# nagadomi/nunif

Measured on AMD Instinct MI355X. Metric: input MPix/s, waifu2x swin_unet 2x tiled render (tile 256) of 1080p frames, higher is better.
Workload: dtype f16; 1 GPU; waifu2x swin_unet 2x (art scale2x geometry), tile_size=256, 1080p frame, random-init weights; tile_size=256, tile_batch=45, tiles_per_frame=45, concurrent_streams=2, parallelism=frame-sharded x1

## Files before the change

### include/nunif_hip.h

```cpp
#ifndef NUNIF_HIP_H
#define NUNIF_HIP_H

#include <stddef.h>
#include <stdint.h>

#ifdef __cplusplus
extern "C" {
#endif

#define NUNIF_HIP_ABI_VERSION 1

typedef enum {
    NUNIF_HIP_OK = 0,
    NUNIF_HIP_EINVAL = -1,
    NUNIF_HIP_ENOMEM = -2,
    NUNIF_HIP_EHIP = -3,
    NUNIF_HIP_EMISSING = -4,
    NUNIF_HIP_EUNSUPPORTED = -5
} nunif_hip_status;

int nunif_hip_abi_version(void);
const char *nunif_hip_last_error(void);

typedef struct {
    int32_t x_h, x_w, scale, offset, tile_size, blend_size;
    int32_t y_h, y_w, h_blocks, w_blocks;
    int32_t pad_l, pad_r, pad_t, pad_b, y_buffer_h, y_buffer_w;
    int32_t input_tile_step, output_tile_step;
    int32_t out_tile_size;
} nunif_tile_grid;

int nunif_hip_tile_grid_init(int32_t x_h, int32_t x_w, int32_t scale, int32_t offset, int32_t tile_size,
                             int32_t blend_size, nunif_tile_grid *grid);

int nunif_hip_blend_ramp(int32_t blend_size, float *ramp );

int nunif_hip_gather_tiles(const float *x, float *tiles, const nunif_tile_grid *grid, int32_t channels,
                           int32_t tile_begin, int32_t n_tiles, void *stream);

int nunif_hip_stitch_tiles(const float *tile_out, float *y, const nunif_tile_grid *grid, int32_t channels,
                           void *stream);

typedef struct {
    const char *name;
    const float *data;
    int32_t ndim;
    int64_t shape[4];
} nunif_tensor_desc;

typedef struct nunif_swin_unet nunif_swin_unet;

int nunif_hip_swin_unet_create(const nunif_tensor_desc *tensors, int32_t n_tensors, int32_t scale_factor,
                               nunif_swin_unet **handle);
void nunif_hip_swin_unet_destroy(nunif_swin_unet *handle);

int nunif_hip_swin_unet_forward(nunif_swin_unet *handle, const float *x, float *z, int32_t batch,
                                int32_t tile_size, void *stream);

int nunif_hip_swin_unet_render(nunif_swin_unet *handle, const float *x, float *y, int32_t x_h, int32_t x_w,
                               int32_t tile_size, int32_t batch_size, void *stream);

int nunif_hip_swin_unet_render_tile_rows(nunif_swin_unet *handle, const float *x, int32_t x_h, int32_t x_w,
                                         int32_t tile_size, int32_t batch_size, int32_t row_begin, int32_t row_end,
                                         void *stream);
int nunif_hip_swin_unet_tile_row_band(nunif_swin_unet *handle, int32_t x_h, int32_t x_w, int32_t tile_size,
                                      int32_t tile_row, int32_t row0, int32_t n_rows, float *band, int32_t import_band,
                                      void *stream);
int nunif_hip_swin_unet_stitch_rows(nunif_swin_unet *handle, float *y_band, int32_t x_h, int32_t x_w, int32_t tile_size,
                                    int32_t y_row_begin, int32_t y_row_end, void *stream);

typedef struct {
    int32_t n_win[2];
    int32_t wrap[2];
} nunif_swin_block_extent;
int nunif_hip_swin_unet_tile_extents(const nunif_tile_grid *grid, int32_t tile_index, const int32_t *blocks_per_stage,
                                     const int32_t *shifts, int32_t to_image_fused, nunif_swin_block_extent *out);

typedef struct {
    int32_t adj[6];
    uint32_t bounds;
    uint32_t reserved;
} nunif_swin_tail_group;
int nunif_hip_swin_unet_tail_groups(const nunif_swin_block_extent *ext, int32_t n_tiles, int32_t S, int32_t shift,
                                    nunif_swin_tail_group *out, int64_t cap, int64_t *n_groups, int64_t *n_tokens);

int nunif_hip_swin_unet_tail192_test(nunif_swin_unet *handle, int32_t stage, int32_t block, const void *att, void *x,
                                     int64_t n_tokens, const nunif_swin_tail_group *groups, int64_t n_groups, int64_t n_listed,
                                     int32_t rev, void *stream);

typedef struct nunif_swin_unet_v2 nunif_swin_unet_v2;
int nunif_hip_swin_unet_v2_create(const nunif_tensor_desc *tensors, int32_t n_tensors, int32_t scale_factor,
                                  nunif_swin_unet_v2 **handle);
void nunif_hip_swin_unet_v2_destroy(nunif_swin_unet_v2 *handle);
int nunif_hip_swin_unet_v2_forward(nunif_swin_unet_v2 *handle, const float *x, float *z, int32_t batch, int32_t tile_size,
                                   int32_t clamp01, void *stream);

typedef struct nunif_cunet nunif_cunet;
int nunif_hip_cunet_create(const nunif_tensor_desc *tensors, int32_t n_tensors, int32_t no_clip, nunif_cunet **handle);
void nunif_hip_cunet_destroy(nunif_cunet *handle);
int nunif_hip_cunet_forward(nunif_cunet *handle, const float *x, float *z, int32_t batch, int32_t tile_size,
                            void *stream);
int nunif_hip_cunet_render(nunif_cunet *handle, const float *x, float *y, int32_t x_h, int32_t x_w,
                           int32_t tile_size, int32_t batch_size, void *stream);

int nunif_hip_tta_view(const float *x, float *y, int32_t C, int32_t H, int32_t W, int32_t view, void *stream);
int nunif_hip_tta_merge(const float *const *views, float *out, int32_t C, int32_t H, int32_t W, void *stream);
int nunif_hip_alpha_border_padding(const float *rgb, const float *alpha, float *out, float *work, int32_t H, int32_t W,
                                   int32_t offset, void *stream);

typedef struct {
    int32_t B, H, W;
    double divergence;
    double convergence;
    int32_t fill;
    int32_t synthetic_view;
    int32_t width_base;
    const float *convergence_dev;
} nunif_forward_warp_params;

int nunif_hip_forward_warp(const float *c, const float *depth, float *left, float *right, float *lmask,
                           float *rmask, const nunif_forward_warp_params *params, void *stream);

typedef struct nunif_depth_anything nunif_depth_anything;
int nunif_hip_depth_anything_create(const nunif_tensor_desc *tensors, int32_t n_tensors, nunif_depth_anything **handle);
int nunif_hip_depth_anything_create_ex(const nunif_tensor_desc *tensors, int32_t n_tensors, const int32_t *taps, float max_depth,
                                       nunif_depth_anything **handle);
void nunif_hip_depth_anything_destroy(nunif_depth_anything *handle);
int nunif_hip_depth_anything_forward(nunif_depth_anything *handle, const float *x, const float *pos, float *depth,
                                     int32_t B, int32_t h, int32_t w, void *stream);
int nunif_hip_depth_anything_reset_state(nunif_depth_anything *handle);
int nunif_hip_depth_anything_is_temporal(const nunif_depth_anything *handle);

typedef struct nunif_da_features {
    const void *outconv;
    const void *bottleneck;
    const void *blocks[4];
    int32_t bh, bw, rh[4], rw[4], channels;
} nunif_da_features;
int nunif_hip_depth_anything_forward_features(nunif_depth_anything *handle, const float *x, const float *pos, float *depth,
                                              int32_t B, int32_t h, int32_t w, nunif_da_features *features, void *stream);

typedef struct nunif_zoedepth_head nunif_zoedepth_head;
int nunif_hip_zoedepth_head_create(const nunif_tensor_desc *tensors, int32_t n_tensors, float alpha, float min_temp, float max_temp,
                                   nunif_zoedepth_head **handle);
int nunif_hip_zoedepth_head_forward(nunif_zoedepth_head *handle, const nunif_da_features *features, const float *rel, float *out,
                                    int32_t B, int32_t h, int32_t w, void *stream);
int nunif_hip_zoedepth_head_debug_taps(nunif_zoedepth_head *handle, int32_t tap, float *dst, int32_t *dims, void *stream);
void nunif_hip_zoedepth_head_destroy(nunif_zoedepth_head *handle);
int nunif_hip_zoedepth_pad_normalize(const float *x, float *y, int64_t planes, int32_t h, int32_t w, int32_t left, int32_t right,
                                     int32_t top, int32_t bottom, void *stream);

typedef struct nunif_depth_aa nunif_depth_aa;
int nunif_hip_depth_aa_create(const nunif_tensor_desc *tensors, int32_t n_tensors, nunif_depth_aa **handle);
void nunif_hip_depth_aa_destroy(nunif_depth_aa *handle);
int nunif_hip_depth_aa_forward(nunif_depth_aa *handle, const float *x, float *y, int32_t B, int32_t h, int32_t w,
                               int32_t mode, void *stream);

typedef struct nunif_row_flow nunif_row_flow;
int nunif_hip_row_flow_create(const nunif_tensor_desc *tensors, int32_t n_tensors, nunif_row_flow **handle);
void nunif_hip_row_flow_destroy(nunif_row_flow *handle);
int nunif_hip_row_flow_delta(nunif_row_flow *handle, const float *x, float *delta, int32_t B, int32_t h, int32_t w,
                             int32_t flip, void *stream);

typedef struct nunif_row_flow_v2 nunif_row_flow_v2;
int nunif_hip_row_flow_v2_create(const nunif_tensor_desc *tensors, int32_t n_tensors, nunif_row_flow_v2 **handle);
void nunif_hip_row_flow_v2_destroy(nunif_row_flow_v2 *handle);
int nunif_hip_row_flow_v2_delta(nunif_row_flow_v2 *handle, const float *x, float *delta, int32_t B, int32_t h, int32_t w,
                                int32_t flip, void *stream);
int nunif_hip_row_flow_v2_debug_taps(nunif_row_flow_v2 *handle, const float *x, float *delta, float *feature, float *relu1,
                                     float *relu2, float *relu3, float *non_overlap, float *residual, int32_t B, int32_t h,
                                     int32_t w, int32_t flip, void *stream);

int nunif_hip_delta_warp(const float *c, const float *delta, float *out, int32_t B, int32_t C, int32_t H, int32_t W,
                         int32_t dh, int32_t dw, double delta_scale, int32_t flip, void *stream);

typedef struct nunif_light_inpaint nunif_light_inpaint;
int nunif_hip_light_inpaint_create(const nunif_tensor_desc *tensors, int32_t n_tensors, nunif_light_inpaint **handle);
void nunif_hip_light_inpaint_destroy(nunif_light_inpaint *handle);
int nunif_hip_light_inpaint_infer(nunif_light_inpaint *handle, const float *x, const uint8_t *mask, float *out, int32_t B,
                                  int32_t H, int32_t W, int32_t closing, int32_t inner_iter, int32_t outer_iter, void *stream);
int nunif_hip_light_inpaint_infer_ex(nunif_light_inpaint *handle, const float *x, const uint8_t *mask, float *out, int32_t B,
                                     int32_t H, int32_t W, int32_t closing, int32_t inner_iter, int32_t outer_iter,
                                     int32_t mirror_x, void *stream);

int nunif_hip_anaglyph(const float *left, const float *right, float *out, int32_t H, int32_t W, int32_t mode, void *stream);
int nunif_hip_equirectangular(const float *c, float *out, int32_t C, int32_t h, int32_t w, void *stream);

typedef struct nunif_mlbw nunif_mlbw;
int nunif_hip_mlbw_create(const nunif_tensor_desc *tensors, int32_t n_tensors, nunif_mlbw **handle);
void nunif_hip_mlbw_destroy(nunif_mlbw *handle);
int32_t nunif_hip_mlbw_num_layers(const nunif_mlbw *handle);
int nunif_hip_mlbw_delta(nunif_mlbw *handle, const float *x, float *delta, float *weight, int32_t B, int32_t h, int32_t w,
                         int32_t flip, void *stream);
int32_t nunif_hip_mlbw_has_hole_mask(const nunif_mlbw *handle);
int nunif_hip_mlbw_delta_mask(nunif_mlbw *handle, const float *x, float *delta, float *weight, float *mask_logits, int32_t B,
                              int32_t h, int32_t w, int32_t flip, void *stream);
int nunif_hip_hole_mask_postprocess(const float *logits, uint8_t *mask, float *work, int32_t B, int32_t h, int32_t w,
                                    int32_t H, int32_t W, float threshold, int32_t inner_iter, int32_t outer_iter, float *z,
                                    int32_t C, void *stream);

int nunif_hip_delta_weight_warp(const float *c, const float *delta, const float *weight, float *out, int32_t B, int32_t C,
                                int32_t H, int32_t W, int32_t dh, int32_t dw, int32_t L, double delta_scale, int32_t flip,
                                void *stream);

int nunif_hip_backward_warp(const float *c, const float *depth, float *left, float *right, int32_t B, int32_t C,
                            int32_t H, int32_t W, int32_t dh, int32_t dw, double divergence, double convergence,
                            int32_t synthetic_view, void *stream, const float *convergence_dev);

int nunif_hip_resize_aa(const float *x, float *y, float *tmp, int64_t planes, int32_t h_in, int32_t w_in,
                        int32_t h_out, int32_t w_out, int32_t bicubic, int32_t align_corners, int32_t clamp01,
                        const float *mean3, const float *std3, void *stream);

int64_t nunif_hip_dilate_edge_work_floats(int32_t B, int32_t H, int32_t W);
int nunif_hip_dilate_edge(const float *x, float *y, float *work, int32_t B, int32_t H, int32_t W, int32_t n_x,
                          int32_t n_y, void *stream);

int nunif_hip_minmax_normalize(const float *x, float *y, float *minmax, int32_t B, int64_t n_per, void *stream);

int nunif_hip_minmax(const float *x, float *minmax_keys, int32_t B, int64_t n_per, void *stream);
int nunif_hip_ema_scaler_push(float *state, const float *minmax_keys, int32_t ring_size, int64_t count, int32_t filled,
                              int32_t first, double decay, void *stream);
int nunif_hip_ema_scaler_ring_minmax(float *state, int32_t ring_size, void *stream);
int nunif_hip_range_normalize(const float *x, float *y, const float *lohi, int64_t n, int32_t max_mode, void *stream);

int nunif_hip_make_input_planes(const float *depth, float *out, int32_t B, int32_t H, int32_t W, double divergence_value,
                                double convergence_value, int32_t border_pix, void *stream, const float *convergence_dev);

int nunif_hip_stack(const void *const *srcs, int32_t n, int64_t bytes_each, void *dst, void *stream);

int nunif_hip_mask_morphology(const float *in, float *out, float *work, int32_t B, int32_t H, int32_t W, int32_t op,
                              int32_t n_a, int32_t n_b, void *stream);

int nunif_hip_reflection_pad2d(const float *x, float *y, int64_t planes, int32_t H, int32_t W, int32_t left, int32_t right,
                               int32_t top, int32_t bottom, void *stream);
int nunif_hip_depth_postprocess(const float *x, float *y, int64_t n, float max_dist, int32_t to_disparity, float eps,
                                int32_t negate, void *stream);

int nunif_hip_frame_to_tensor(const void *frame, float *chw, int32_t H, int32_t W, int32_t bits, void *stream);
int nunif_hip_stereo_to_frame(const float *left, const float *right, void *frame, int32_t H, int32_t W,
                              int32_t layout, int32_t bits, void *stream);
int nunif_hip_stereo_compose(const float *left, const float *right, float *out, int32_t H, int32_t W,
                             int32_t layout, void *stream);

int nunif_hip_rgb_noise(float *out, int32_t planes, int32_t H, int32_t W, int32_t level, int32_t component, uint64_t seed,
                        uint64_t counter, void *stream);
int nunif_hip_apply_rgb_noise(const float *rgb, const float *noise, float *out, int64_t n, double strength, double gamma,
                              int32_t light_decay, double light_decay_strength, void *stream);
int nunif_hip_grain_blend(float *buf, const float *noise, int64_t n, double speed, int32_t first, void *stream);
int nunif_hip_grain_video_step(const float *rgb, float *noise_buffer, void *frame, int32_t H, int32_t W, int32_t bits,
                               int32_t level, uint64_t seed, uint64_t counter, double speed, int32_t first, double strength,
                               double gamma, int32_t light_decay, double light_decay_strength, void *stream);
int nunif_hip_frame_to_tensor_rot(const void *frame, float *chw, int32_t H, int32_t W, int32_t bits, int32_t turns,
                                  void *stream);

int nunif_hip_map_depth(const float *x, float *y, int64_t n, int32_t kind, double p0, double p1, void *stream);

typedef struct nunif_transnetv2 nunif_transnetv2;
int nunif_hip_transnetv2_create(const nunif_tensor_desc *tensors, int32_t n_tensors, int32_t filters,
                                nunif_transnetv2 **handle);
void nunif_hip_transnetv2_destroy(nunif_transnetv2 *handle);
int nunif_hip_transnetv2_forward(nunif_transnetv2 *handle, const float *frames, int32_t B, int32_t T, float *one_hot,
                                 float *many_hot, float *sigmoid_out, void *stream);

typedef struct nunif_sod_v1 nunif_sod_v1;
int nunif_hip_sod_v1_create(const nunif_tensor_desc *tensors, int32_t n_tensors, int32_t net_size, nunif_sod_v1 **handle);
void nunif_hip_sod_v1_destroy(nunif_sod_v1 *handle);
int64_t nunif_hip_sod_v1_workspace_floats(int32_t B);
int nunif_hip_sod_v1_forward(nunif_sod_v1 *handle, const float *rgb, int32_t H, int32_t W, const float *depth, int32_t h,
                             int32_t w, int32_t B, float *workspace, float *saliency, float *depth_scaled, void *stream);
int nunif_hip_sod_v1_entry(const float *rgb, int32_t H, int32_t W, const float *depth, int32_t h, int32_t w, int32_t B,
                           float *x6, float *depth_scaled, void *stream);
int nunif_hip_sod_v1_debug_taps(nunif_sod_v1 *handle, const float *workspace, int32_t B, const char *name, float *out,
                                int64_t capacity, int64_t *shape4, void *stream);
int nunif_hip_sod_v1_depth_position(const float *saliency, const float *depth, int32_t B, int64_t n, double pos, float *out,
                                    void *stream);
int nunif_hip_sod_v1_ema(const float *z, float *out, int32_t B, float *state, double decay, uint64_t reset_mask, void *stream);

typedef struct nunif_superpoint nunif_superpoint;
int nunif_hip_superpoint_create(const nunif_tensor_desc *tensors, int32_t n_tensors, nunif_superpoint **handle);
void nunif_hip_superpoint_destroy(nunif_superpoint *handle);
int nunif_hip_superpoint_forward(nunif_superpoint *handle, const float *image, int32_t B, int32_t C, int32_t H, int32_t W,
                                 int32_t nms_radius, int32_t remove_borders, float threshold, float *keypoints,
                                 float *kp_scores, int32_t *counts, void *stream);
int nunif_hip_superpoint_debug_taps(nunif_superpoint *handle, const char *name, float *out, int64_t capacity, int64_t *shape4,
                                    void *stream);
int nunif_hip_superpoint_sample(nunif_superpoint *handle, int32_t b, const float *keypoints, int32_t n, float *out,
                                void *stream);

int64_t nunif_hip_superpoint_keypoints_work_floats(int32_t B, int32_t H, int32_t W);
int nunif_hip_superpoint_keypoints(const float *scores, int32_t B, int32_t H, int32_t W, int32_t nms_radius,
                                   int32_t remove_borders, float threshold, float *work, float *nms_out, float *keypoints,
                                   float *kp_scores, int32_t *counts, void *stream);

int nunif_hip_sample_descriptors(const float *keypoints, int32_t n, const float *dense, int32_t h, int32_t w, int32_t C,
                                 int32_t stride, float *out, void *stream);

int nunif_hip_superpoint_match(const float *d1, int32_t n1, const float *d2, int32_t n2, int32_t D, void *work, int64_t *index,
                               float *max_similarity, void *stream);

int nunif_hip_affine_warp(const float *x, const float *params, float *out, int32_t B, int32_t C, int32_t H, int32_t W,
                          int32_t padding_mode, void *stream);

typedef struct nunif_outpaint nunif_outpaint;
int nunif_hip_outpaint_create(const nunif_tensor_desc *tensors, int32_t n_tensors, nunif_outpaint **handle);
void nunif_hip_outpaint_destroy(nunif_outpaint *handle);
int64_t nunif_hip_outpaint_work_bytes(int32_t B, int32_t H, int32_t W, int32_t max_size);
int nunif_hip_outpaint_infer(nunif_outpaint *handle, const float *x, const uint8_t *mask, int32_t B, int32_t H, int32_t W,
                             int32_t max_size, int32_t mode, float *out, void *work, void *stream);
int nunif_hip_outpaint_debug_taps(nunif_outpaint *handle, const void *work, int32_t B, int32_t H, int32_t W, int32_t max_size,
                                  const char *name, float *out, int64_t capacity, int64_t *shape4, void *stream);
int nunif_hip_outpaint_buffer_step(const float *frames, const float *coarse, float *buffer, const uint8_t *reset,
                                   double buffer_decay, int32_t B, int32_t H, int32_t W, float *out, uint8_t *mask0,
                                   void *stream);

int nunif_hip_autocrop_stats(const float *x, int32_t B, int32_t H, int32_t W, int32_t flat, int32_t passes,
                             int32_t *border_count_tb, int32_t *border_count_lr, void *work, int64_t work_bytes, void *stream);
int nunif_hip_autocrop_debug_stats(const float *x, int32_t B, int32_t H, int32_t W, int32_t flat, int32_t passes,
                                   int32_t *border_count_tb, int32_t *border_count_lr, void *work, int64_t work_bytes,
                                   float *row_a, float *row_b, float *col_a, float *col_b, void *stream);
int nunif_hip_autocrop_crop_pad(const float *src, float *dst, int64_t N, int32_t sH, int32_t sW, int32_t dH, int32_t dW,
                                int32_t y0, int32_t x0, int32_t pad_top, int32_t pad_left, int32_t win_h, int32_t win_w,
                                float pad_value, void *stream);

int nunif_hip_jpeg_quant_tables(int32_t quality, uint8_t *luma, uint8_t *chroma);
int64_t nunif_hip_jpeg_header(int32_t H, int32_t W, int32_t quality, int32_t subsampling, int32_t restart_mcus, uint8_t *out,
                              int64_t capacity);
int64_t nunif_hip_jpeg_max_bytes(int32_t H, int32_t W, int32_t subsampling, int32_t restart_mcus);
int64_t nunif_hip_jpeg_workspace_bytes(int32_t B, int32_t H, int32_t W, int32_t subsampling, int32_t restart_mcus);
int nunif_hip_jpeg_encode(const float *rgb, int32_t B, int32_t H, int32_t W, int32_t quality, int32_t subsampling,
                          int32_t restart_mcus, uint8_t *out, int64_t capacity, int32_t *out_len, void *workspace, void *stream);
int nunif_hip_jpeg_debug_coefficients(const float *rgb, int32_t B, int32_t H, int32_t W, int32_t quality, int32_t subsampling,
                                      int16_t *coef, void *stream);

typedef struct nunif_hdr2sdr_params {
    double exposure, white_point, saturation_gain;
} nunif_hdr2sdr_params;
int nunif_hip_hdr2sdr(const void *src, void *dst, int32_t H, int32_t W, int32_t trc, int32_t colorspace,
                      const nunif_hdr2sdr_params *params, int32_t form, void *stream);
int nunif_hip_hdr2sdr_constants(int32_t trc, int32_t colorspace, const nunif_hdr2sdr_params *params, float *matrix,
                                float *hable_white);

typedef struct nunif_pixfmt_planes {
    void *data[3];
    int64_t pitch[3];
} nunif_pixfmt_planes;
int nunif_hip_yuv_to_tensor(const nunif_pixfmt_planes *src, int32_t format, int32_t H, int32_t W, int32_t matrix,
                            int32_t full_range, int32_t form, float *dst, void *frame, void *stream);
int nunif_hip_tensor_to_yuv(const float *src, int32_t H, int32_t W, int32_t format, int32_t matrix, int32_t full_range,
                            const nunif_pixfmt_planes *dst, void *stream);
int nunif_hip_pixfmt_constants(int32_t matrix, int32_t full_range, int32_t bits, int32_t direction, float *coefficients,
                               float *offsets);

int nunif_hip_yuv_hdr_to_tensor(const nunif_pixfmt_planes *src, int32_t format, int32_t H, int32_t W, int32_t full_range,
                                int32_t trc, int32_t colorspace, const nunif_hdr2sdr_params *params, int32_t form,
                                void *dst, void *stream);

typedef struct nunif_cliqa nunif_cliqa;
int nunif_hip_cliqa_create(const nunif_tensor_desc *tensors, int32_t n_tensors, int32_t kind, nunif_cliqa **handle);
void nunif_hip_cliqa_destroy(nunif_cliqa *handle);
int64_t nunif_hip_cliqa_workspace_bytes(nunif_cliqa *handle, int32_t B, int32_t H, int32_t W, int32_t group);
int nunif_hip_cliqa_forward(nunif_cliqa *handle, const float *x, int32_t B, int32_t H, int32_t W, int32_t group, void *workspace,
                            int64_t workspace_bytes, float *out0, float *out1, void *stream);
int nunif_hip_cliqa_debug_taps(nunif_cliqa *handle, const float *x, int32_t B, int32_t H, int32_t W, int32_t group,
                               void *workspace, int64_t workspace_bytes, float *out0, float *out1, void *tap1, void *tap2,
                               void *tap3, float *head_maps, void *stream);
int nunif_hip_cliqa_select_patches(const float *image, int32_t H, int32_t W, int32_t patch_size, int32_t num_patches,
                                   float *scores, int64_t *indices, float *patches, void *stream);

int64_t nunif_hip_png_header(int32_t H, int32_t W, int32_t form, const char *const *text_keys, const char *const *text_values,
                             int32_t n_text, uint8_t *out, int64_t capacity);
int64_t nunif_hip_png_max_bytes(int32_t H, int32_t W, int32_t form, int32_t stripe_rows);
int64_t nunif_hip_png_workspace_bytes(int32_t B, int32_t H, int32_t W, int32_t form, int32_t stripe_rows);
int nunif_hip_png_encode(const void *src, int32_t form, int32_t B, int32_t H, int32_t W, int32_t stripe_rows, uint8_t *out,
                         int64_t capacity, int32_t *out_len, void *workspace, void *stream);
int nunif_hip_png_debug_filtered(const void *src, int32_t form, int32_t B, int32_t H, int32_t W, uint8_t *filtered, void *stream);
int nunif_hip_png_debug_codes(const void *src, int32_t form, int32_t B, int32_t H, int32_t W, int32_t stripe_rows, int32_t *hist,
                              int32_t *lengths, void *workspace, void *stream);
int nunif_hip_png_encode_planes(const float *colour, const float *alpha, int32_t colour_channels, int32_t form, int32_t B, int32_t H,
                                int32_t W, int32_t stripe_rows, uint8_t *out, int64_t capacity, int32_t *out_len, void *workspace,
                                void *stream);
int nunif_hip_png_debug_filtered_planes(const float *colour, const float *alpha, int32_t colour_channels, int32_t form, int32_t B,
                                        int32_t H, int32_t W, uint8_t *filtered, void *stream);

int64_t nunif_hip_da3_disparity_workspace_bytes(int32_t B, int32_t H, int32_t W);
int nunif_hip_da3_disparity(const float *depth, const float *sky, int32_t B, int32_t H, int32_t W, double sky_thresh, double shift,
                            int32_t raw_output, float *out, void *workspace, int64_t workspace_bytes, void *stream);
int nunif_hip_da3_disparity_debug_stats(const void *workspace, int32_t B, float *stats, int32_t *counts, void *stream);
int64_t nunif_hip_da3mono_features_workspace_bytes(int32_t B, int32_t H, int32_t W);
int nunif_hip_da3mono_features(const float *depth, int32_t B, int32_t H, int32_t W, const int64_t *ranks, float *out,
                               void *workspace, int64_t workspace_bytes, void *stream);
typedef struct nunif_da3mono nunif_da3mono;
int nunif_hip_da3mono_create(const nunif_tensor_desc *tensors, int32_t n_tensors, nunif_da3mono **handle);
void nunif_hip_da3mono_destroy(nunif_da3mono *handle);
int64_t nunif_hip_da3mono_workspace_bytes(int32_t B, int32_t H, int32_t W);
int nunif_hip_da3mono_forward(nunif_da3mono *handle, const float *depth, int32_t B, int32_t H, int32_t W, const int64_t *ranks,
                              float *out, void *workspace, int64_t workspace_bytes, void *stream);

int nunif_hip_swin_unet_debug_taps(nunif_swin_unet *handle, int32_t enable);
int nunif_hip_swin_unet_get_tap(nunif_swin_unet *handle, int32_t index, char *name, int32_t name_cap,
                                void *host_dst, int64_t cap_bytes, int64_t *nbytes);
int nunif_hip_cunet_debug_taps(nunif_cunet *handle, int32_t enable);
int nunif_hip_cunet_get_tap(nunif_cunet *handle, int32_t index, char *name, int32_t name_cap,
                            void *host_dst, int64_t cap_bytes, int64_t *nbytes);

int nunif_hip_profile_enable(int32_t on);
typedef struct { char name[48]; double total_ms; int64_t launches; double flops; double bytes; } nunif_prof_record;
int nunif_hip_profile_read(nunif_prof_record *out, int32_t cap, int32_t reset);

#ifdef __cplusplus
}
#endif
#endif
```

### nunif_amd/_hip.py

```python
import ctypes
import os

_HERE = os.path.dirname(os.path.abspath(__file__))
LIB_PATH = os.environ.get("NUNIF_HIP_LIB") or os.path.join(_HERE, "libnunif_hip.so")

c_void_p, c_int32, c_int64, c_float, c_char_p, c_double, c_uint64 = (
    ctypes.c_void_p, ctypes.c_int32, ctypes.c_int64, ctypes.c_float, ctypes.c_char_p, ctypes.c_double, ctypes.c_uint64)


class NunifHipError(RuntimeError):
    def __init__(self, status, message):
        super().__init__(f"libnunif_hip error {status}: {message}")
        self.status = status


class TileGrid(ctypes.Structure):
    _fields_ = [(n, c_int32) for n in (
        "x_h", "x_w", "scale", "offset", "tile_size", "blend_size",
        "y_h", "y_w", "h_blocks", "w_blocks",
        "pad_l", "pad_r", "pad_t", "pad_b", "y_buffer_h", "y_buffer_w",
        "input_tile_step", "output_tile_step", "out_tile_size")]

    def as_config(self):
        return {"y_h": self.y_h, "y_w": self.y_w, "h_blocks": self.h_blocks, "w_blocks": self.w_blocks,
                "pad": (self.pad_l, self.pad_r, self.pad_t, self.pad_b),
                "y_buffer_h": self.y_buffer_h, "y_buffer_w": self.y_buffer_w,
                "input_tile_step": self.input_tile_step, "output_tile_step": self.output_tile_step}


class SwinBlockExtent(ctypes.Structure):
    _fields_ = [("n_win", c_int32 * 2), ("wrap", c_int32 * 2)]


class SwinTailGroup(ctypes.Structure):
    _fields_ = [("adj", c_int32 * 6), ("bounds", ctypes.c_uint32), ("reserved", ctypes.c_uint32)]

    def tokens(self):
        cnt = (self.bounds >> 25) & 31
        firsts = [0] + [(self.bounds >> (5 * p)) & 31 for p in range(5)]
        return [self.adj[max(p for p in range(6) if firsts[p] <= r)] + r for r in range(cnt)]


class TensorDesc(ctypes.Structure):
    _fields_ = [("name", c_char_p), ("data", c_void_p), ("ndim", c_int32), ("shape", c_int64 * 4)]


class ForwardWarpParams(ctypes.Structure):
    _fields_ = [("B", c_int32), ("H", c_int32), ("W", c_int32), ("divergence", c_double), ("convergence", c_double),
                ("fill", c_int32), ("synthetic_view", c_int32), ("width_base", c_int32), ("convergence_dev", c_void_p)]


class Hdr2SdrParams(ctypes.Structure):
    _fields_ = [("exposure", c_double), ("white_point", c_double), ("saturation_gain", c_double)]


class PixfmtPlanes(ctypes.Structure):
    _fields_ = [("data", c_void_p * 3), ("pitch", c_int64 * 3)]


class DaFeatures(ctypes.Structure):
    _fields_ = [("outconv", c_void_p), ("bottleneck", c_void_p), ("blocks", c_void_p * 4), ("bh", c_int32), ("bw", c_int32),
                ("rh", c_int32 * 4), ("rw", c_int32 * 4), ("channels", c_int32)]


class ProfRecord(ctypes.Structure):
    _fields_ = [("name", ctypes.c_char * 48), ("total_ms", c_double), ("launches", c_int64),
                ("flops", c_double), ("bytes", c_double)]


SIGNATURES = {
    "nunif_hip_abi_version": (c_int32, []),
    "nunif_hip_last_error": (c_char_p, []),
    "nunif_hip_tile_grid_init": (c_int32, [c_int32] * 6 + [ctypes.POINTER(TileGrid)]),
    "nunif_hip_blend_ramp": (c_int32, [c_int32, ctypes.POINTER(c_float)]),
    "nunif_hip_gather_tiles": (c_int32, [c_void_p, c_void_p, ctypes.POINTER(TileGrid), c_int32, c_int32, c_int32, c_void_p]),
    "nunif_hip_stitch_tiles": (c_int32, [c_void_p, c_void_p, ctypes.POINTER(TileGrid), c_int32, c_void_p]),
    "nunif_hip_swin_unet_create": (c_int32, [ctypes.POINTER(TensorDesc), c_int32, c_int32, ctypes.POINTER(c_void_p)]),
    "nunif_hip_swin_unet_destroy": (None, [c_void_p]),
    "nunif_hip_swin_unet_forward": (c_int32, [c_void_p, c_void_p, c_void_p, c_int32, c_int32, c_void_p]),
    "nunif_hip_swin_unet_render": (c_int32, [c_void_p, c_void_p, c_void_p, c_int32, c_int32, c_int32, c_int32, c_void_p]),
    "nunif_hip_swin_unet_render_tile_rows": (c_int32, [c_void_p, c_void_p, c_int32, c_int32, c_int32, c_int32, c_int32, c_int32, c_void_p]),
    "nunif_hip_swin_unet_tile_row_band": (c_int32, [c_void_p, c_int32, c_int32, c_int32, c_int32, c_int32, c_int32, c_void_p, c_int32, c_void_p]),
    "nunif_hip_swin_unet_stitch_rows": (c_int32, [c_void_p, c_void_p, c_int32, c_int32, c_int32, c_int32, c_int32, c_void_p]),
    "nunif_hip_swin_unet_tile_extents": (c_int32, [ctypes.POINTER(TileGrid), c_int32, ctypes.POINTER(c_int32), ctypes.POINTER(c_int32),
                                                   c_int32, ctypes.POINTER(SwinBlockExtent)]),
    "nunif_hip_swin_unet_tail_groups": (c_int32, [ctypes.POINTER(SwinBlockExtent), c_int32, c_int32, c_int32,
                                                  ctypes.POINTER(SwinTailGroup), c_int64, ctypes.POINTER(c_int64), ctypes.POINTER(c_int64)]),
    "nunif_hip_swin_unet_tail192_test": (c_int32, [c_void_p, c_int32, c_int32, c_void_p, c_void_p, c_int64, c_void_p, c_int64, c_int64,
                                                   c_int32, c_void_p]),
    "nunif_hip_swin_unet_v2_create": (c_int32, [ctypes.POINTER(TensorDesc), c_int32, c_int32, ctypes.POINTER(c_void_p)]),
    "nunif_hip_swin_unet_v2_destroy": (None, [c_void_p]),
    "nunif_hip_swin_unet_v2_forward": (c_int32, [c_void_p, c_void_p, c_void_p, c_int32, c_int32, c_int32, c_void_p]),
    "nunif_hip_cunet_create": (c_int32, [ctypes.POINTER(TensorDesc), c_int32, c_int32, ctypes.POINTER(c_void_p)]),
    "nunif_hip_cunet_destroy": (None, [c_void_p]),
    "nunif_hip_cunet_forward": (c_int32, [c_void_p, c_void_p, c_void_p, c_int32, c_int32, c_void_p]),
    "nunif_hip_cunet_render": (c_int32, [c_void_p, c_void_p, c_void_p, c_int32, c_int32, c_int32, c_int32, c_void_p]),
    "nunif_hip_forward_warp": (c_int32, [c_void_p, c_void_p, c_void_p, c_void_p, c_void_p, c_void_p,
                                         ctypes.POINTER(ForwardWarpParams), c_void_p]),
    "nunif_hip_backward_warp": (c_int32, [c_void_p, c_void_p, c_void_p, c_void_p] + [c_int32] * 6 +
                                [c_double, c_double, c_int32, c_void_p, c_void_p]),
    "nunif_hip_row_flow_create": (c_int32, [ctypes.POINTER(TensorDesc), c_int32, ctypes.POINTER(c_void_p)]),
    "nunif_hip_row_flow_destroy": (None, [c_void_p]),
    "nunif_hip_row_flow_delta": (c_int32, [c_void_p, c_void_p, c_void_p, c_int32, c_int32, c_int32, c_int32, c_void_p]),
    "nunif_hip_row_flow_v2_create": (c_int32, [ctypes.POINTER(TensorDesc), c_int32, ctypes.POINTER(c_void_p)]),
    "nunif_hip_row_flow_v2_destroy": (None, [c_void_p]),
    "nunif_hip_row_flow_v2_delta": (c_int32, [c_void_p, c_void_p, c_void_p, c_int32, c_int32, c_int32, c_int32, c_void_p]),
    "nunif_hip_row_flow_v2_debug_taps": (c_int32, [c_void_p] * 9 + [c_int32] * 4 + [c_void_p]),
    "nunif_hip_delta_warp": (c_int32, [c_void_p, c_void_p, c_void_p] + [c_int32] * 6 + [c_double, c_int32, c_void_p]),
    "nunif_hip_mlbw_create": (c_int32, [ctypes.POINTER(TensorDesc), c_int32, ctypes.POINTER(c_void_p)]),
    "nunif_hip_mlbw_destroy": (None, [c_void_p]),
    "nunif_hip_mlbw_num_layers": (c_int32, [c_void_p]),
    "nunif_hip_mlbw_delta": (c_int32, [c_void_p, c_void_p, c_void_p, c_void_p, c_int32, c_int32, c_int32, c_int32, c_void_p]),
    "nunif_hip_light_inpaint_create": (c_int32, [ctypes.POINTER(TensorDesc), c_int32, ctypes.POINTER(c_void_p)]),
    "nunif_hip_light_inpaint_destroy": (None, [c_void_p]),
    "nunif_hip_light_inpaint_infer": (c_int32, [c_void_p, c_void_p, c_void_p, c_void_p] + [c_int32] * 6 + [c_void_p]),
    "nunif_hip_light_inpaint_infer_ex": (c_int32, [c_void_p, c_void_p, c_void_p, c_void_p] + [c_int32] * 7 + [c_void_p]),
    "nunif_hip_anaglyph": (c_int32, [c_void_p, c_void_p, c_void_p, c_int32, c_int32, c_int32, c_void_p]),
    "nunif_hip_equirectangular": (c_int32, [c_void_p, c_void_p, c_int32, c_int32, c_int32, c_void_p]),
    "nunif_hip_mlbw_has_hole_mask": (c_int32, [c_void_p]),
    "nunif_hip_mlbw_delta_mask": (c_int32, [c_void_p, c_void_p, c_void_p, c_void_p, c_void_p, c_int32, c_int32, c_int32, c_int32,
                                            c_void_p]),
    "nunif_hip_hole_mask_postprocess": (c_int32, [c_void_p, c_void_p, c_void_p] + [c_int32] * 5 + [c_float, c_int32, c_int32,
                                                  c_void_p, c_int32, c_void_p]),
    "nunif_hip_delta_weight_warp": (c_int32, [c_void_p, c_void_p, c_void_p, c_void_p] + [c_int32] * 7 +
                                    [c_double, c_int32, c_void_p]),
    "nunif_hip_depth_aa_create": (c_int32, [ctypes.POINTER(TensorDesc), c_int32, ctypes.POINTER(c_void_p)]),
    "nunif_hip_depth_aa_destroy": (None, [c_void_p]),
    "nunif_hip_depth_aa_forward": (c_int32, [c_void_p, c_void_p, c_void_p, c_int32, c_int32, c_int32, c_int32, c_void_p]),
    "nunif_hip_depth_anything_create": (c_int32, [ctypes.POINTER(TensorDesc), c_int32, ctypes.POINTER(c_void_p)]),
    "nunif_hip_depth_anything_create_ex": (c_int32, [ctypes.POINTER(TensorDesc), c_int32, ctypes.POINTER(c_int32), ctypes.c_float,
                                                     ctypes.POINTER(c_void_p)]),
    "nunif_hip_depth_anything_destroy": (None, [c_void_p]),
    "nunif_hip_depth_anything_forward": (c_int32, [c_void_p, c_void_p, c_void_p, c_void_p, c_int32, c_int32, c_int32, c_void_p]),
    "nunif_hip_depth_anything_reset_state": (c_int32, [c_void_p]),
    "nunif_hip_depth_anything_is_temporal": (c_int32, [c_void_p]),
    "nunif_hip_depth_anything_forward_features": (c_int32, [c_void_p, c_void_p, c_void_p, c_void_p, c_int32, c_int32, c_int32,
                                                            ctypes.POINTER(DaFeatures), c_void_p]),
    "nunif_hip_zoedepth_head_create": (c_int32, [ctypes.POINTER(TensorDesc), c_int32, c_float, c_float, c_float,
                                                 ctypes.POINTER(c_void_p)]),
    "nunif_hip_zoedepth_head_forward": (c_int32, [c_void_p, ctypes.POINTER(DaFeatures), c_void_p, c_void_p, c_int32, c_int32,
                                                  c_int32, c_void_p]),
    "nunif_hip_zoedepth_head_debug_taps": (c_int32, [c_void_p, c_int32, c_void_p, ctypes.POINTER(c_int32), c_void_p]),
    "nunif_hip_zoedepth_head_destroy": (None, [c_void_p]),
    "nunif_hip_zoedepth_pad_normalize": (c_int32, [c_void_p, c_void_p, c_int64] + [c_int32] * 6 + [c_void_p]),
    "nunif_hip_tta_view": (c_int32, [c_void_p, c_void_p, c_int32, c_int32, c_int32, c_int32, c_void_p]),
    "nunif_hip_tta_merge": (c_int32, [ctypes.POINTER(c_void_p), c_void_p, c_int32, c_int32, c_int32, c_void_p]),
    "nunif_hip_alpha_border_padding": (c_int32, [c_void_p, c_void_p, c_void_p, c_void_p, c_int32, c_int32, c_int32, c_void_p]),
    "nunif_hip_resize_aa": (c_int32, [c_void_p, c_void_p, c_void_p, c_int64] + [c_int32] * 7 +
                            [ctypes.POINTER(c_float), ctypes.POINTER(c_float), c_void_p]),
    "nunif_hip_dilate_edge": (c_int32, [c_void_p, c_void_p, c_void_p] + [c_int32] * 5 + [c_void_p]),
    "nunif_hip_dilate_edge_work_floats": (ctypes.c_int64, [c_int32, c_int32, c_int32]),
    "nunif_hip_minmax_normalize": (c_int32, [c_void_p, c_void_p, c_void_p, c_int32, c_int64, c_void_p]),
    "nunif_hip_mask_morphology": (c_int32, [c_void_p, c_void_p, c_void_p] + [c_int32] * 6 + [c_void_p]),
    "nunif_hip_reflection_pad2d": (c_int32, [c_void_p, c_void_p, c_int64, c_int32, c_int32, c_int32, c_int32, c_int32, c_int32,
                                             c_void_p]),
    "nunif_hip_depth_postprocess": (c_int32, [c_void_p, c_void_p, c_int64, c_float, c_int32, c_float, c_int32, c_void_p]),
    "nunif_hip_frame_to_tensor": (c_int32, [c_void_p, c_void_p, c_int32, c_int32, c_int32, c_void_p]),
    "nunif_hip_stereo_to_frame": (c_int32, [c_void_p, c_void_p, c_void_p, c_int32, c_int32, c_int32, c_int32, c_void_p]),
    "nunif_hip_stereo_compose": (c_int32, [c_void_p, c_void_p, c_void_p, c_int32, c_int32, c_int32, c_void_p]),
    "nunif_hip_rgb_noise": (c_int32, [c_void_p, c_int32, c_int32, c_int32, c_int32, c_int32, c_uint64, c_uint64, c_void_p]),
    "nunif_hip_apply_rgb_noise": (c_int32, [c_void_p, c_void_p, c_void_p, c_int64, c_double, c_double, c_int32, c_double, c_void_p]),
    "nunif_hip_grain_blend": (c_int32, [c_void_p, c_void_p, c_int64, c_double, c_int32, c_void_p]),
    "nunif_hip_grain_video_step": (c_int32, [c_void_p, c_void_p, c_void_p, c_int32, c_int32, c_int32, c_int32, c_uint64, c_uint64,
                                             c_double, c_int32, c_double, c_double, c_int32, c_double, c_void_p]),
    "nunif_hip_frame_to_tensor_rot": (c_int32, [c_void_p, c_void_p, c_int32, c_int32, c_int32, c_int32, c_void_p]),
    "nunif_hip_map_depth": (c_int32, [c_void_p, c_void_p, c_int64, c_int32, c_double, c_double, c_void_p]),
    "nunif_hip_transnetv2_create": (c_int32, [ctypes.POINTER(TensorDesc), c_int32, c_int32, ctypes.POINTER(c_void_p)]),
    "nunif_hip_transnetv2_destroy": (None, [c_void_p]),
    "nunif_hip_transnetv2_forward": (c_int32, [c_void_p, c_void_p, c_int32, c_int32, c_void_p, c_void_p, c_void_p, c_void_p]),
    "nunif_hip_sod_v1_create": (c_int32, [ctypes.POINTER(TensorDesc), c_int32, c_int32, ctypes.POINTER(c_void_p)]),
    "nunif_hip_sod_v1_destroy": (None, [c_void_p]),
    "nunif_hip_sod_v1_workspace_floats": (c_int64, [c_int32]),
    "nunif_hip_sod_v1_forward": (c_int32, [c_void_p, c_void_p, c_int32, c_int32, c_void_p, c_int32, c_int32, c_int32, c_void_p,
                                           c_void_p, c_void_p, c_void_p]),
    "nunif_hip_sod_v1_entry": (c_int32, [c_void_p, c_int32, c_int32, c_void_p, c_int32, c_int32, c_int32, c_void_p, c_void_p,
                                         c_void_p]),
    "nunif_hip_sod_v1_debug_taps": (c_int32, [c_void_p, c_void_p, c_int32, c_char_p, c_void_p, c_int64, ctypes.POINTER(c_int64),
                                              c_void_p]),
    "nunif_hip_sod_v1_depth_position": (c_int32, [c_void_p, c_void_p, c_int32, c_int64, c_double, c_void_p, c_void_p]),
    "nunif_hip_sod_v1_ema": (c_int32, [c_void_p, c_void_p, c_int32, c_void_p, c_double, c_uint64, c_void_p]),
    "nunif_hip_superpoint_create": (c_int32, [ctypes.POINTER(TensorDesc), c_int32, ctypes.POINTER(c_void_p)]),
    "nunif_hip_superpoint_destroy": (None, [c_void_p]),
    "nunif_hip_superpoint_forward": (c_int32, [c_void_p, c_void_p] + [c_int32] * 6 + [c_float, c_void_p, c_void_p, c_void_p,
                                              c_void_p]),
    "nunif_hip_superpoint_debug_taps": (c_int32, [c_void_p, c_char_p, c_void_p, c_int64, ctypes.POINTER(c_int64), c_void_p]),
    "nunif_hip_superpoint_sample": (c_int32, [c_void_p, c_int32, c_void_p, c_int32, c_void_p, c_void_p]),
    "nunif_hip_superpoint_keypoints_work_floats": (c_int64, [c_int32, c_int32, c_int32]),
    "nunif_hip_superpoint_keypoints": (c_int32, [c_void_p] + [c_int32] * 5 + [c_float] + [c_void_p] * 6),
    "nunif_hip_sample_descriptors": (c_int32, [c_void_p, c_int32, c_void_p] + [c_int32] * 4 + [c_void_p, c_void_p]),
    "nunif_hip_superpoint_match": (c_int32, [c_void_p, c_int32, c_void_p, c_int32, c_int32, c_void_p, c_void_p, c_void_p,
                                            c_void_p]),
    "nunif_hip_affine_warp": (c_int32, [c_void_p, c_void_p, c_void_p] + [c_int32] * 5 + [c_void_p]),
    "nunif_hip_outpaint_create": (c_int32, [ctypes.POINTER(TensorDesc), c_int32, ctypes.POINTER(c_void_p)]),
    "nunif_hip_outpaint_destroy": (None, [c_void_p]),
    "nunif_hip_outpaint_work_bytes": (c_int64, [c_int32] * 4),
    "nunif_hip_outpaint_infer": (c_int32, [c_void_p, c_void_p, c_void_p] + [c_int32] * 5 + [c_void_p, c_void_p, c_void_p]),
    "nunif_hip_outpaint_debug_taps": (c_int32, [c_void_p, c_void_p] + [c_int32] * 4 + [c_char_p, c_void_p, c_int64,
                                                ctypes.POINTER(c_int64), c_void_p]),
    "nunif_hip_outpaint_buffer_step": (c_int32, [c_void_p] * 4 + [c_double] + [c_int32] * 3 + [c_void_p] * 3),
    "nunif_hip_autocrop_stats": (c_int32, [c_void_p] + [c_int32] * 5 + [c_void_p, c_void_p, c_void_p, c_int64, c_void_p]),
    "nunif_hip_autocrop_debug_stats": (c_int32, [c_void_p] + [c_int32] * 5 + [c_void_p, c_void_p, c_void_p, c_int64] +
                                       [c_void_p] * 5),
    "nunif_hip_autocrop_crop_pad": (c_int32, [c_void_p, c_void_p, c_int64] + [c_int32] * 10 + [c_float, c_void_p]),
    "nunif_hip_jpeg_quant_tables": (c_int32, [c_int32, c_void_p, c_void_p]),
    "nunif_hip_jpeg_header": (c_int64, [c_int32] * 5 + [c_void_p, c_int64]),
    "nunif_hip_jpeg_max_bytes": (c_int64, [c_int32] * 4),
    "nunif_hip_jpeg_workspace_bytes": (c_int64, [c_int32] * 5),
    "nunif_hip_jpeg_encode": (c_int32, [c_void_p] + [c_int32] * 6 + [c_void_p, c_int64, c_void_p, c_void_p, c_void_p]),
    "nunif_hip_jpeg_debug_coefficients": (c_int32, [c_void_p] + [c_int32] * 5 + [c_void_p, c_void_p]),
    "nunif_hip_png_header": (c_int64, [c_int32] * 3 + [c_void_p, c_void_p, c_int32, c_void_p, c_int64]),
    "nunif_hip_png_max_bytes": (c_int64, [c_int32] * 4),
    "nunif_hip_png_workspace_bytes": (c_int64, [c_int32] * 5),
    "nunif_hip_png_encode": (c_int32, [c_void_p] + [c_int32] * 5 + [c_void_p, c_int64, c_void_p, c_void_p, c_void_p]),
    "nunif_hip_png_debug_filtered": (c_int32, [c_void_p] + [c_int32] * 4 + [c_void_p, c_void_p]),
    "nunif_hip_png_debug_codes": (c_int32, [c_void_p] + [c_int32] * 5 + [c_void_p] * 4),
    "nunif_hip_png_encode_planes": (c_int32, [c_void_p, c_void_p] + [c_int32] * 6 + [c_void_p, c_int64, c_void_p, c_void_p, c_void_p]),
    "nunif_hip_png_debug_filtered_planes": (c_int32, [c_void_p, c_void_p] + [c_int32] * 5 + [c_void_p, c_void_p]),
    "nunif_hip_hdr2sdr": (c_int32, [c_void_p, c_void_p, c_int32, c_int32, c_int32, c_int32, ctypes.POINTER(Hdr2SdrParams), c_int32,
                                    c_void_p]),
    "nunif_hip_hdr2sdr_constants": (c_int32, [c_int32, c_int32, ctypes.POINTER(Hdr2SdrParams), ctypes.POINTER(c_float),
                                              ctypes.POINTER(c_float)]),
    "nunif_hip_yuv_to_tensor": (c_int32, [ctypes.POINTER(PixfmtPlanes)] + [c_int32] * 6 + [c_void_p, c_void_p, c_void_p]),
    "nunif_hip_tensor_to_yuv": (c_int32, [c_void_p] + [c_int32] * 5 + [ctypes.POINTER(PixfmtPlanes), c_void_p]),
    "nunif_hip_pixfmt_constants": (c_int32, [c_int32] * 4 + [ctypes.POINTER(c_float), ctypes.POINTER(c_float)]),
    "nunif_hip_yuv_hdr_to_tensor": (c_int32, [ctypes.POINTER(PixfmtPlanes)] + [c_int32] * 6 + [ctypes.POINTER(Hdr2SdrParams), c_int32,
                                                                                                c_void_p, c_void_p]),
    "nunif_hip_cliqa_create": (c_int32, [ctypes.POINTER(TensorDesc), c_int32, c_int32, ctypes.POINTER(c_void_p)]),
    "nunif_hip_cliqa_destroy": (None, [c_void_p]),
    "nunif_hip_cliqa_workspace_bytes": (c_int64, [c_void_p] + [c_int32] * 4),
    "nunif_hip_cliqa_forward": (c_int32, [c_void_p, c_void_p] + [c_int32] * 4 + [c_void_p, c_int64] + [c_void_p] * 3),
    "nunif_hip_cliqa_debug_taps": (c_int32, [c_void_p, c_void_p] + [c_int32] * 4 + [c_void_p, c_int64] + [c_void_p] * 7),
    "nunif_hip_cliqa_select_patches": (c_int32, [c_void_p] + [c_int32] * 4 + [c_void_p] * 4),
    "nunif_hip_da3_disparity_workspace_bytes": (c_int64, [c_int32] * 3),
    "nunif_hip_da3_disparity": (c_int32, [c_void_p, c_void_p] + [c_int32] * 3 + [c_double, c_double, c_int32, c_void_p, c_void_p,
                                                                                 c_int64, c_void_p]),
    "nunif_hip_da3_disparity_debug_stats": (c_int32, [c_void_p, c_int32, c_void_p, c_void_p, c_void_p]),
    "nunif_hip_da3mono_features_workspace_bytes": (c_int64, [c_int32] * 3),
    "nunif_hip_da3mono_features": (c_int32, [c_void_p] + [c_int32] * 3 + [c_void_p, c_void_p, c_void_p, c_int64, c_void_p]),
    "nunif_hip_da3mono_create": (c_int32, [ctypes.POINTER(TensorDesc), c_int32, ctypes.POINTER(c_void_p)]),
    "nunif_hip_da3mono_destroy": (None, [c_void_p]),
    "nunif_hip_da3mono_workspace_bytes": (c_int64, [c_int32] * 3),
    "nunif_hip_da3mono_forward": (c_int32, [c_void_p, c_void_p] + [c_int32] * 3 + [c_void_p, c_void_p, c_void_p, c_int64, c_void_p]),
    "nunif_hip_swin_unet_debug_taps":(c_int32, [c_void_p, c_int32]),
    "nunif_hip_swin_unet_get_tap": (c_int32, [c_void_p, c_int32, c_char_p, c_int32, c_void_p, c_int64,
                                              ctypes.POINTER(c_int64)]),
    "nunif_hip_cunet_debug_taps": (c_int32, [c_void_p, c_int32]),
    "nunif_hip_cunet_get_tap": (c_int32, [c_void_p, c_int32, c_char_p, c_int32, c_void_p, c_int64,
                                          ctypes.POINTER(c_int64)]),
    "nunif_hip_minmax": (c_int32, [c_void_p, c_void_p, c_int32, c_int64, c_void_p]),
    "nunif_hip_ema_scaler_push": (c_int32, [c_void_p, c_void_p, c_int32, c_int64, c_int32, c_int32, c_double, c_void_p]),
    "nunif_hip_ema_scaler_ring_minmax": (c_int32, [c_void_p, c_int32, c_void_p]),
    "nunif_hip_range_normalize": (c_int32, [c_void_p, c_void_p, c_void_p, c_int64, c_int32, c_void_p]),
    "nunif_hip_make_input_planes": (c_int32, [c_void_p, c_void_p, c_int32, c_int32, c_int32, c_double, c_double, c_int32, c_void_p, c_void_p]),
    "nunif_hip_stack": (c_int32, [ctypes.POINTER(c_void_p), c_int32, c_int64, c_void_p, c_void_p]),
    "nunif_hip_profile_enable": (c_int32, [c_int32]),
    "nunif_hip_profile_read": (c_int32, [ctypes.POINTER(ProfRecord), c_int32, c_int32]),
}

_lib = None


def lib():
    global _lib
    if _lib is None:
        import torch
        if not os.path.exists(LIB_PATH):
            raise RuntimeError(
                f"{LIB_PATH} not found: the HIP engine is not built. Run `python -m nunif_amd.build` "
                "(there is no CPU fallback).")
        handle = ctypes.CDLL(LIB_PATH)
        for name, (restype, argtypes) in SIGNATURES.items():
            fn = getattr(handle, name)
            fn.restype = restype
            fn.argtypes = argtypes
        _lib = handle
    return _lib


def check(status):
    if status != 0:
        raise NunifHipError(status, lib().nunif_hip_last_error().decode("utf-8", "replace"))


def current_stream_ptr(device=None):
    import torch
    return c_void_p(torch.cuda.current_stream(device).cuda_stream)


def tile_grid(x_h, x_w, scale, offset, tile_size, blend_size):
    g = TileGrid()
    check(lib().nunif_hip_tile_grid_init(x_h, x_w, scale, offset, tile_size, blend_size or 0, ctypes.byref(g)))
    return g


def swin_tile_extents(grid, tile_index, blocks_per_stage=(2, 2, 6, 2, 2), shifts=None, to_image_fused=True):
    n = sum(blocks_per_stage)
    if shifts is None:
        shifts = [3 if i % 2 else 0 for k in blocks_per_stage for i in range(k)]
    per = (c_int32 * 5)(*blocks_per_stage)
    sh = (c_int32 * n)(*shifts)
    out = (SwinBlockExtent * n)()
    check(lib().nunif_hip_swin_unet_tile_extents(ctypes.byref(grid), tile_index, per, sh, 1 if to_image_fused else 0, out))
    return [(e.n_win[0], e.n_win[1], e.wrap[0], e.wrap[1]) for e in out]


def swin_tail_groups(extents, S, shift):
    ext = (SwinBlockExtent * len(extents))()
    for e, (ny, nx, wy, wx) in zip(ext, extents):
        e.n_win[0], e.n_win[1], e.wrap[0], e.wrap[1] = ny, nx, wy, wx
    ng, nt = c_int64(0), c_int64(0)
    check(lib().nunif_hip_swin_unet_tail_groups(ext, len(extents), S, shift, None, 0, ctypes.byref(ng), ctypes.byref(nt)))
    out = (SwinTailGroup * max(1, ng.value))()
    if ng.value:
        check(lib().nunif_hip_swin_unet_tail_groups(ext, len(extents), S, shift, out, ng.value, ctypes.byref(ng), ctypes.byref(nt)))
    return (SwinTailGroup * ng.value).from_buffer(out) if ng.value else (SwinTailGroup * 0)(), nt.value


def blend_ramp(blend_size):
    buf = (c_float * max(1, blend_size))()
    check(lib().nunif_hip_blend_ramp(blend_size, buf))
    return list(buf)[:blend_size]


def profile_enable(on=True):
    check(lib().nunif_hip_profile_enable(1 if on else 0))


def profile_read(reset=True):
    recs = (ProfRecord * 64)()
    n = lib().nunif_hip_profile_read(recs, 64, 1 if reset else 0)
    return [{"name": recs[i].name.decode(), "total_ms": recs[i].total_ms, "launches": recs[i].launches,
             "flops": recs[i].flops, "bytes": recs[i].bytes} for i in range(n)]
```

### nunif_amd/csrc/swin_kernels.h

```cpp
#pragma once
#include "common.h"

namespace nunif {

struct GemmArgs {
    const f16 *a; int B, Hi, Wi, Cin;
    int Ho, Wo, stride, oy, ox, kw;
    int K;
    const f16 *w;
    const float *bias;
    int N;
    int mode;
    int act;
    float slope;
    const f16 *res;
    void *out;
    int ldo;
    int n_real;
    int ps;
    int oshift, OH, OW;
    int no_clamp;
    int lda;
    int rev;
    int nt_chunk;
    int res_H = 0, res_W = 0, res_crop = 0;
    const float *in_scale = nullptr;
};
int launch_gemm(const GemmArgs &g, hipStream_t s, const char *tag);

struct PatchUpArgs { const f16 *a, *w; const float *bias; const f16 *res; f16 *out; int B, Ho, Wo, Cq, rev; };
bool patchup_supported(const PatchUpArgs &g);
int launch_patchup(const PatchUpArgs &g, hipStream_t s);

struct PatchDownArgs { const f16 *a, *w; const float *bias; f16 *out; int B, Ho, Wo, Cin, oy, rev; int N = 192; int act = 0; float slope = 0.f; };
bool patchdown_supported(const PatchDownArgs &g);
int launch_patchdown(const PatchDownArgs &g, hipStream_t s);

struct CunetUpArgs { const f16 *a, *w; const float *bias; const f16 *res; f16 *out; const float *in_scale; int B, S, res_S, crop;
                     float slope; };
bool cunet_up_supported(const CunetUpArgs &g);
int launch_cunet_up(const CunetUpArgs &g, hipStream_t s);

struct GemmOsArgs {
    const f16 *a; long M; int lda, K;
    const f16 *w; const float *bias; int N;
    int act;
    const f16 *res;
    f16 *out; int ldo;
    float2 *stats_out;
    const float2 *stats_in; int stats_parts; const float *wsum; float ln_eps;
};
bool gemm_os_supported(long M, int N, int K);
bool gemm_os_consumes_stats(long M, int N, int K);
int launch_gemm_os(const GemmOsArgs &g, hipStream_t s, const char *tag);

struct DaMlpArgs {
    f16 *t; long M;
    const f16 *w1; const float *b1, *ws1;
    const f16 *w2c; const float *b2;
    const float2 *stats_in; float2 *stats_out; float ln_eps;
    void *partial; unsigned *flags;
};
bool da_mlp_supported(int D, int hidden);

struct CunetHeadArgs { const f16 *a, *w; const float *bias; float *out32; const float *add32; int B, Hi, Wi, Ho, Wo, addH, addW, add_crop, clamp01; };
bool cunet_head_supported(const CunetHeadArgs &g);
int launch_cunet_head(const CunetHeadArgs &g, hipStream_t s);

constexpr int kVdaGnBlocks = 256;
int launch_vda_groupnorm(const f16 *x, const float *gamma, const float *beta, f16 *y, float2 *part, int frames, int P, int C, float eps, hipStream_t s);
int launch_vda_layernorm(const f16 *x, const float *gamma, const float *beta, f16 *y, long T, int C, float eps, hipStream_t s);
int launch_vda_geglu(const f16 *h, f16 *out, long T, int I, hipStream_t s);
struct VdaTattnArgs { const f16 *qkv; f16 *kc, *vc; const float *pq, *pk, *pv; f16 *att; int P, C, hd, start, idx; };
int launch_vda_tattn(const VdaTattnArgs &g, hipStream_t s);
long da_mlp_partial_bytes(long M);
long da_mlp_flag_count(long M);
int launch_da_mlp(const DaMlpArgs &a, hipStream_t s);

struct Stem1Args {
    const float *x;
    int frame_mode, H, W, wb, istep, pad_t, pad_l, tile_begin;
    int B, T;
    const float *w;
    const float *bias;
    int C1, C1P;
    f16 *out;
    float slope;
};
int launch_stem1(const Stem1Args &a, hipStream_t s);

struct StemFusedArgs {
    const float *x;
    int frame_mode, H, W, wb, istep, pad_t, pad_l, tile_begin;
    int B, T;
    const f16 *w1;
    const f16 *w2;
    const float *b2;
    f16 *out;
    float slope;
    int rev;
    int C1, C, crop;
};
bool stem_fused_supported(int C1, int C);
int launch_stem_fused(const StemFusedArgs &a, hipStream_t s);

int proj_mlp_stream_frags(int C);
struct TailToImage { const f16 *w; const float *bias; float *out; int H, W, ps, n_real; };
struct WinMap { int on, H, W, shift; const int *pixmap; };
int launch_winmap_build(int *pixmap, int B, int H, int W, int shift, hipStream_t s);
int launch_winmap_list_build(int *pixmap, const unsigned *win_list, int n_list, int H, int W, int shift, hipStream_t s);
int launch_proj_mlp(const f16 *att, f16 *x, const f16 *wstream, const float *bp, const float *b0, const float *b3,
                    long M, int C, hipStream_t s, const TailToImage *to_image = nullptr, int rev = 0,
                    const WinMap *wm = nullptr, int gelu32 = 0);

int swin_block96_tail_frags();
int swin_block96_btab_floats();
int launch_swin_block96(f16 *x, const f16 *wqkv, const float *bqkv, const float *btab, const f16 *wtail, const float *bp,
                        const float *b0, const float *b3, int B, int H, int W, int shift, hipStream_t s,
                        const TailToImage *ti = nullptr, int rev = 0);

int proj_mlp_ws_stream_frags();
int launch_proj_mlp_ws(const f16 *att, f16 *x, const f16 *wws, const float *bp, const float *b0, const float *b3, long M,
                       hipStream_t s, int rev = 0, int gelu32 = 0, const nunif_swin_tail_group *groups = nullptr, long n_groups = 0,
                       long n_listed = 0);

constexpr int kQkvBiasFloatsPerHead = 36 * 52;
int launch_qkv_attn_r(const f16 *x, f16 *att, const f16 *wres, const float *bqkv, const float *btab32,
                      int B, int H, int W, int C, int heads, int shift, hipStream_t s, int rev = 0, int window_major = 0,
                      const unsigned *win_list = nullptr, int n_list = 0);

int launch_window_attn(const f16 *qkv, f16 *out, const float *bias, int B, int H, int W, int heads, int hd,
                       int shift, hipStream_t s);

int launch_layernorm_nobias(const f16 *x, f16 *y, const float *gamma, long M, int C, hipStream_t s);

struct ConvArgs {
    const f16 *a; const f16 *a2;
    int H2, W2, crop2;
    int B, Hi, Wi, Cin, Ho, Wo, stride, kh, kw;
    const f16 *wstream;
    const float *bias;
    int N, n_real;
    int act; float slope;
    f16 *out;
    float *out32;
    const float *add32; int addH, addW, add_crop;
    int clamp01;
    int rpad;
    const f16 *res;
    int zpad;
    int relu_in;
    const f16 *res2;
    int ldo;
    int cmaj;
    float *part32;
};
long gemm_big_m();
int launch_conv(const ConvArgs &g, hipStream_t s);
bool conv3_lds_applies(const ConvArgs &g);
int launch_conv3_lds(const ConvArgs &g, hipStream_t s);
bool conv3_dma_applies(const ConvArgs &g);
int launch_conv3_dma(const ConvArgs &g, hipStream_t s);

struct C3ConvArgs {
    const float *x; int frame_mode, H, W, wb, istep, pad_t, pad_l, tile_begin;
    int B, T;
    const float *w, *bias;
    int C;
    f16 *out;
    float slope;
};
int launch_c3_conv(const C3ConvArgs &a, hipStream_t s);

int launch_se(f16 *x, float *sums, float *scale, const float *w1, const float *b1, const float *w2, const float *b2,
              int B, long hw, int C, hipStream_t s, int scale_in_consumer = 0);

}
```

### nunif_amd/csrc/swin_patchdown.hip

```cpp
#include <algorithm>
#include <cstdlib>

#include "swin_kernels.h"

namespace nunif {

namespace {
constexpr int kWaves = 8;
constexpr int kMF = 2;
}

template <int CIN, int kKS, int kNT, bool LRELU>
__global__ void __launch_bounds__(kWaves * 64) patchdown_kernel(PatchDownArgs g) {
    static_assert(CIN == 64 || CIN == 96 || CIN == 192, "Cin");
    constexpr int kWBytes = kNT * kKS * 1024;
    extern __shared__ __attribute__((aligned(1024))) unsigned char smem_pd[];
    const f16x8 *wres = reinterpret_cast<const f16x8 *>(smem_pd);
    const float4 *bres = reinterpret_cast<const float4 *>(smem_pd + kWBytes);
    const int tid = threadIdx.x, lane = tid & 63, r16 = lane & 15, grp = lane >> 4;
    const int wave = __builtin_amdgcn_readfirstlane(tid >> 6);
    {
        const unsigned char *src = reinterpret_cast<const unsigned char *>(g.w) + lane * 16;
        const unsigned lds0 = (unsigned)reinterpret_cast<size_t>(smem_pd);
#pragma unroll
        for (int u = 0; u < kWBytes / 1024 / kWaves; ++u) {
            const int i = wave + kWaves * u;
            dma16(src + (size_t)i * 1024, lds0 + i * 1024);
        }
        if (tid < kNT * 4) reinterpret_cast<float4 *>(smem_pd + kWBytes)[tid] = reinterpret_cast<const float4 *>(g.bias)[tid];
    }
    const unsigned Wo = (unsigned)g.Wo, Ho = (unsigned)g.Ho, Wi = 2 * Wo, Hi = 2 * Ho;
    const unsigned M = (unsigned)g.B * Ho * Wo;
    const unsigned n_groups = (M + kMF * 16 - 1) / (kMF * 16);
    const unsigned step = gridDim.x * kWaves;
    unsigned gi = blockIdx.x * kWaves + wave;
    const bool any = gi < n_groups;
    const int prc = pair_run_channel(grp);

    struct Grp { unsigned in[kMF], out[kMF]; };
    auto coords = [&](unsigned gidx, Grp &c) {
        const unsigned gg = g.rev ? n_groups - 1 - gidx : gidx;
#pragma unroll
        for (int f = 0; f < kMF; ++f) {
            unsigned m = gg * (kMF * 16) + f * 16 + r16;
            m = m < M ? m : M - 1;
            const unsigned t = m / Wo, x = m - t * Wo;
            const unsigned b = t / Ho, y = t - b * Ho;
            c.in[f] = (((b * Hi + 2 * y + (unsigned)g.oy) * Wi + 2 * x) * CIN + grp * 8) * 2;
            c.out[f] = (m * (kNT * 16) + prc) * 2;
        }
    };
    auto ks_off = [&](int ks) -> unsigned {
        const int k0 = ks * 32, tap = k0 / CIN, c0 = k0 % CIN;
        const int dy = tap / 2, dx = tap % 2;
        return (unsigned)((dy * Wi + dx) * CIN + c0) * 2;
    };
    auto load_frag = [&](const Grp &c, int f, int ks) -> f16x8 {
        const unsigned char *base = reinterpret_cast<const unsigned char *>(g.a) + (size_t)ks_off(ks);
        return *reinterpret_cast<const f16x8 *>(base + (size_t)c.in[f]);
    };

    Grp cur, nxt;
    f16x8 xf[kMF][kKS];
    coords(any ? gi : 0, cur);
#pragma unroll
    for (int ks = 0; ks < kKS; ++ks) {
#pragma unroll
        for (int f = 0; f < kMF; ++f) xf[f][ks] = load_frag(cur, f, ks);
    }
    asm volatile("s_waitcnt vmcnt(0)" ::: "memory");
#pragma unroll
    for (int ks = 0; ks < kKS; ++ks) {
#pragma unroll
        for (int f = 0; f < kMF; ++f) asm volatile("" : "+v"(xf[f][ks]));
    }
    __syncthreads();
    if (!any) return;

    while (true) {
        const unsigned gn = gi + step;
        const bool has_next = gn < n_groups;
        coords(has_next ? gn : gi, nxt);
        int lofs = lane;
        asm volatile("" : "+v"(lofs));
        f32x4 acc[kNT][kMF];
#pragma unroll
        for (int nt = 0; nt < kNT; ++nt) {
            const float4 bv = bres[nt * 4 + (lofs >> 4)];
#pragma unroll
            for (int f = 0; f < kMF; ++f) acc[nt][f] = (f32x4){bv.x, bv.y, bv.z, bv.w};
        }
#pragma unroll
        for (int ks = 0; ks < kKS; ++ks) {
#pragma unroll
            for (int nt = 0; nt < kNT; ++nt) {
                const f16x8 wv = wres[(nt * kKS + ks) * 64 + lofs];
#pragma unroll
                for (int f = 0; f < kMF; ++f) acc[nt][f] = MFMA_16x16x32(wv, xf[f][ks], acc[nt][f]);
            }
#pragma unroll
            for (int f = 0; f < kMF; ++f) xf[f][ks] = load_frag(nxt, f, ks);
            __builtin_amdgcn_sched_barrier(0);
        }
        unsigned char *obase = reinterpret_cast<unsigned char *>(g.out);
#pragma unroll
        for (int p = 0; p < kNT / 2; ++p) {
#pragma unroll
            for (int f = 0; f < kMF; ++f) {
                f32x4 a0 = acc[2 * p][f], a1 = acc[2 * p + 1][f];
                if constexpr (LRELU) {
#pragma unroll
                    for (int r = 0; r < 4; ++r) {
                        a0[r] = a0[r] >= 0.f ? a0[r] : a0[r] * g.slope;
                        a1[r] = a1[r] >= 0.f ? a1[r] : a1[r] * g.slope;
                    }
                }
                const f16x8 ov = pair_to_run((f16x4){(f16)a0[0], (f16)a0[1], (f16)a0[2], (f16)a0[3]},
                                             (f16x4){(f16)a1[0], (f16)a1[1], (f16)a1[2], (f16)a1[3]});
                *reinterpret_cast<f16x8 *>(obase + (size_t)cur.out[f] + p * 64) = ov;
            }
        }
        if (!has_next) break;
        cur = nxt;
        gi = gn;
    }
}

bool patchdown_supported(const PatchDownArgs &g) {
    if (const char *e = getenv("NUNIF_PATCHDOWN")) if (atoi(e) == 0) return false;
    const long M = (long)g.B * g.Ho * g.Wo;
    const bool shape = (g.Cin == 96 && g.N == 192 && g.oy == 0) || (g.Cin == 192 && g.N == 192 && (g.oy == 0 || g.oy == 1)) ||
                       (g.Cin == 64 && g.N == 64 && g.oy == 0);
    const bool act_ok = g.Cin == 64 ? g.act == 2 : g.act == 0;
    return shape && M > 0 && 4 * M * g.Cin * 2 < (1L << 32) && M * g.N * 2 < (1L << 32) && act_ok;
}

template <int CIN, int KS, int NT, bool LRELU>
static int launch_pd(const PatchDownArgs &g, hipStream_t s, const char *name, int wgs_per_cu) {
    constexpr int smem = NT * KS * 1024 + NT * 16 * 4;
    static_assert(smem <= 160 * 1024, "LDS");
    const long M = (long)g.B * g.Ho * g.Wo;
    static bool configured = false;
    static int cus = 256;
    if (!configured) {
        NUNIF_HIP_CHECK(hipFuncSetAttribute((const void *)patchdown_kernel<CIN, KS, NT, LRELU>, hipFuncAttributeMaxDynamicSharedMemorySize, smem));
        int dev = 0;
        NUNIF_HIP_CHECK(hipGetDevice(&dev));
        NUNIF_HIP_CHECK(hipDeviceGetAttribute(&cus, hipDeviceAttributeMultiprocessorCount, dev));
        configured = true;
    }
    const long groups = (M + kMF * 16 - 1) / (kMF * 16);
    const unsigned grid = (unsigned)std::max<long>(1, std::min<long>((groups + kWaves - 1) / kWaves, (long)cus * wgs_per_cu));
    ProfScope ps(name, s, 2.0 * (double)M * (KS * 32.0) * (NT * 16.0), (double)M * (KS * 32.0 + NT * 16.0) * 2.0);
    patchdown_kernel<CIN, KS, NT, LRELU><<<grid, kWaves * 64, smem, s>>>(g);
    NUNIF_LAUNCH_CHECK();
    return NUNIF_HIP_OK;
}

int launch_patchdown(const PatchDownArgs &g, hipStream_t s) {
    NUNIF_REQUIRE(g.a && g.w && g.bias && g.out && patchdown_supported(g), "patchdown: bad argument");
    if (g.Cin == 96) return launch_pd<96, 12, 12, false>(g, s, "patchdown_kernel<96>", 1);
    if (g.Cin == 192) return launch_pd<192, 12, 12, false>(g, s, "patchdown_kernel<192>", 1);
    return launch_pd<64, 8, 4, true>(g, s, "patchdown_kernel<64>", 2);
}

}
```

### nunif_amd/csrc/swin_patchup.hip

```cpp
#include <algorithm>
#include <cstdlib>

#include "swin_kernels.h"

namespace nunif {

namespace {
constexpr int kKS = 6;
constexpr int kNT = 24;
constexpr int kTrips = kNT / 2;
constexpr int kWaves = 8;
constexpr int kMF = 2;
#ifndef NUNIF_PU_KD
#define NUNIF_PU_KD 4
#endif
constexpr int kD = NUNIF_PU_KD;
constexpr int kWBytes = kNT * kKS * 1024;
constexpr int kSmem = kWBytes + 384 * 4;
static_assert(kSmem <= 160 * 1024, "LDS");
static_assert(kTrips % kD == 0, "the ring slot of a trip is static");
}

template <int CQ>
__global__ void __launch_bounds__(kWaves * 64) patchup_kernel(PatchUpArgs g) {
    constexpr int HALVES = 4 * CQ / (kNT * 16);
    static_assert(HALVES == 1 || HALVES == 2, "Cq is 96 or 192");
    extern __shared__ __attribute__((aligned(1024))) unsigned char smem_pu[];
    const f16x8 *wres = reinterpret_cast<const f16x8 *>(smem_pu);
    const float4 *bres = reinterpret_cast<const float4 *>(smem_pu + kWBytes);
    const int tid = threadIdx.x, lane = tid & 63, r16 = lane & 15, grp = lane >> 4;
    const int wave = __builtin_amdgcn_readfirstlane(tid >> 6);
    const int half = HALVES == 2 ? (int)(blockIdx.x & 1) : 0;
    const unsigned wb = blockIdx.x / HALVES, nwb = gridDim.x / HALVES;

    {
        const unsigned char *src = reinterpret_cast<const unsigned char *>(g.w) + (size_t)half * kWBytes + lane * 16;
        const unsigned lds0 = (unsigned)reinterpret_cast<size_t>(smem_pu);
#pragma unroll
        for (int u = 0; u < kWBytes / 1024 / kWaves; ++u) {
            const int i = wave + kWaves * u;
            dma16(src + (size_t)i * 1024, lds0 + i * 1024);
        }
        if (tid < 96) reinterpret_cast<float4 *>(smem_pu + kWBytes)[tid] = reinterpret_cast<const float4 *>(g.bias + half * 384)[tid];
    }

    const unsigned Wo = (unsigned)g.Wo, Ho = (unsigned)g.Ho;
    const unsigned M = (unsigned)g.B * Ho * Wo;
    const unsigned n_groups = (M + kMF * 16 - 1) / (kMF * 16);
    const unsigned step = nwb * kWaves;
    unsigned gi = wb * kWaves + wave;
    const bool any = gi < n_groups;
    const int prc = pair_run_channel(grp);

    auto trip_off = [&](int t) -> unsigned {
        const int ql = (t * 32) / CQ, c = (t * 32) % CQ;
        const int q = HALVES == 2 ? 2 * half + ql : ql;
        return (unsigned)(((q >> 1) * 2 * Wo + (q & 1)) * CQ + c);
    };
    struct Grp { unsigned pix[kMF], xo[kMF]; };
    auto coords = [&](unsigned gidx, Grp &c) {
        const unsigned gg = g.rev ? n_groups - 1 - gidx : gidx;
#pragma unroll
        for (int f = 0; f < kMF; ++f) {
            unsigned m = gg * (kMF * 16) + f * 16 + r16;
            m = m < M ? m : M - 1;
            const unsigned t = m / Wo, x = m - t * Wo;
            const unsigned b = t / Ho, y = t - b * Ho;
            c.xo[f] = (m * (kKS * 32) + grp * 8) * 2;
            c.pix[f] = (((b * 2 * Ho + 2 * y) * (2 * Wo) + 2 * x) * CQ + prc) * 2;
        }
    };
    auto load_x = [&](const Grp &c, f16x8 (&xf)[kMF][kKS]) {
#pragma unroll
        for (int f = 0; f < kMF; ++f) {
            const unsigned char *p = reinterpret_cast<const unsigned char *>(g.a) + (size_t)c.xo[f];
#pragma unroll
            for (int ks = 0; ks < kKS; ++ks) xf[f][ks] = *reinterpret_cast<const f16x8 *>(p + ks * 64);
        }
    };
    auto load_res = [&](const Grp &c, int t, f16x8 (&r)[kMF]) {
        const unsigned char *base = reinterpret_cast<const unsigned char *>(g.res) + (size_t)trip_off(t) * 2;
#pragma unroll
        for (int f = 0; f < kMF; ++f) r[f] = *reinterpret_cast<const f16x8 *>(base + (size_t)c.pix[f]);
    };

    Grp cur, nxt;
    f16x8 xc[kMF][kKS], xn[kMF][kKS];
    f16x8 rr[kD][kMF];
    coords(any ? gi : 0, cur);
    load_x(cur, xc);
#pragma unroll
    for (int t = 0; t < kD; ++t) load_res(cur, t, rr[t]);
    asm volatile("s_waitcnt vmcnt(0)" ::: "memory");
#pragma unroll
    for (int f = 0; f < kMF; ++f) {
#pragma unroll
        for (int ks = 0; ks < kKS; ++ks) asm volatile("" : "+v"(xc[f][ks]));
#pragma unroll
        for (int t = 0; t < kD; ++t) asm volatile("" : "+v"(rr[t][f]));
    }
    __syncthreads();
    if (!any) return;

    while (true) {
        const unsigned gn = gi + step;
        const bool has_next = gn < n_groups;
        coords(has_next ? gn : gi, nxt);
        load_x(nxt, xn);
        int lofs = lane;
        asm volatile("" : "+v"(lofs));
#pragma unroll
        for (int t = 0; t < kTrips; ++t) {
            f32x4 acc0[kMF], acc1[kMF];
            {
                const float4 b0 = bres[t * 8 + (lofs >> 4)], b1 = bres[t * 8 + 4 + (lofs >> 4)];
#pragma unroll
                for (int f = 0; f < kMF; ++f) {
                    acc0[f] = (f32x4){b0.x, b0.y, b0.z, b0.w};
                    acc1[f] = (f32x4){b1.x, b1.y, b1.z, b1.w};
                }
            }
            f16x8 wa[kKS], wb[kKS];
#pragma unroll
            for (int ks = 0; ks < kKS; ++ks) wa[ks] = wres[((2 * t) * kKS + ks) * 64 + lofs];
#pragma unroll
            for (int ks = 0; ks < kKS; ++ks) wb[ks] = wres[((2 * t + 1) * kKS + ks) * 64 + lofs];
#pragma unroll
            for (int ks = 0; ks < kKS; ++ks) {
#pragma unroll
                for (int f = 0; f < kMF; ++f) acc0[f] = MFMA_16x16x32(wa[ks], xc[f][ks], acc0[f]);
            }
#pragma unroll
            for (int ks = 0; ks < kKS; ++ks) {
#pragma unroll
                for (int f = 0; f < kMF; ++f) acc1[f] = MFMA_16x16x32(wb[ks], xc[f][ks], acc1[f]);
            }
            unsigned char *obase = reinterpret_cast<unsigned char *>(g.out) + (size_t)trip_off(t) * 2;
#pragma unroll
            for (int f = 0; f < kMF; ++f) asm volatile("" : "+v"(rr[t % kD][f]));
#pragma unroll
            for (int f = 0; f < kMF; ++f) {
                float lo[4], hi[4];
#pragma unroll
                for (int r = 0; r < 4; ++r) {
                    const float a0 = acc0[f][r], a1 = acc1[f][r];
                    const u32x2 sw = lane16_swap(__builtin_bit_cast(unsigned, a0), __builtin_bit_cast(unsigned, a1));
                    const unsigned s0 = sw[0], s1 = sw[1];
                    lo[r] = __builtin_bit_cast(float, s0);
                    hi[r] = __builtin_bit_cast(float, s1);
                }
                const f16x8 rv = rr[t % kD][f];
                f16x8 ov;
#pragma unroll
                for (int r = 0; r < 4; ++r) {
                    ov[r] = (f16)(lo[r] + (float)rv[r]);
                    ov[4 + r] = (f16)(hi[r] + (float)rv[4 + r]);
                }
                *reinterpret_cast<f16x8 *>(obase + (size_t)cur.pix[f]) = ov;
            }
            if (t + kD < kTrips) load_res(cur, t + kD, rr[t % kD]);
            else load_res(nxt, t + kD - kTrips, rr[t % kD]);
        }
        if (!has_next) break;
#pragma unroll
        for (int f = 0; f < kMF; ++f) {
#pragma unroll
            for (int ks = 0; ks < kKS; ++ks) xc[f][ks] = xn[f][ks];
        }
        cur = nxt;
        gi = gn;
    }
}

bool patchup_supported(const PatchUpArgs &g) {
    if (const char *e = getenv("NUNIF_PATCHUP")) if (atoi(e) == 0) return false;
    const long M = (long)g.B * g.Ho * g.Wo;
    return (g.Cq == 96 || g.Cq == 192) && g.res && M > 0 && M * 384 < (1L << 32) && M * 8 * g.Cq < (1L << 32);
}

int launch_patchup(const PatchUpArgs &g, hipStream_t s) {
    NUNIF_REQUIRE(g.a && g.w && g.bias && g.res && g.out && patchup_supported(g), "patchup: bad argument");
    const long M = (long)g.B * g.Ho * g.Wo;
    static bool configured = false;
    static int cus = 256;
    if (!configured) {
        NUNIF_HIP_CHECK(hipFuncSetAttribute((const void *)patchup_kernel<96>, hipFuncAttributeMaxDynamicSharedMemorySize, kSmem));
        NUNIF_HIP_CHECK(hipFuncSetAttribute((const void *)patchup_kernel<192>, hipFuncAttributeMaxDynamicSharedMemorySize, kSmem));
        int dev = 0;
        NUNIF_HIP_CHECK(hipGetDevice(&dev));
        NUNIF_HIP_CHECK(hipDeviceGetAttribute(&cus, hipDeviceAttributeMultiprocessorCount, dev));
        configured = true;
    }
    const long groups = (M + kMF * 16 - 1) / (kMF * 16);
    const int halves = g.Cq == 192 ? 2 : 1;
    const long per_half = std::max<long>(1, std::min<long>((groups + kWaves - 1) / kWaves, std::max(1, cus / halves)));
    const unsigned grid = (unsigned)(per_half * halves);
    const double flops = 2.0 * (double)M * 192.0 * 4.0 * g.Cq;
    const double bytes = (double)M * (192.0 * 2.0 + 4.0 * g.Cq * 2.0 * 2.0);
    if (g.Cq == 96) {
        ProfScope ps("patchup_kernel<96>", s, flops, bytes);
        patchup_kernel<96><<<grid, kWaves * 64, kSmem, s>>>(g);
    } else {
        ProfScope ps("patchup_kernel<192>", s, flops, bytes);
        patchup_kernel<192><<<grid, kWaves * 64, kSmem, s>>>(g);
    }
    NUNIF_LAUNCH_CHECK();
    return NUNIF_HIP_OK;
}

}
```

### nunif_amd/csrc/swin_unet.cpp

```cpp
#include <algorithm>
#include <cmath>
#include <cstdlib>
#include <cstring>
#include <list>
#include <string>
#include <vector>

#include "host_weights.h"
#include "swin_kernels.h"
#include "swin_tail_groups_host.h"

namespace nunif {

int launch_stitch(const float *tile_out, float *y, const nunif_tile_grid *g, int C, hipStream_t s, int y0 = 0, int rows = -1,
                  int compact = 0);

namespace {

struct Linear {
    f16 *w = nullptr;
    float *bias = nullptr;
    int N = 0, n_real = 0, K = 0;
};

struct Block {
    Linear qkv, proj, mlp0, mlp3;
    Linear mlp0p, mlp3p;
    float *norm1 = nullptr, *norm2 = nullptr;
    bool fast = true;
    float *attn_bias = nullptr;
    f16 *tail_stream = nullptr;
    f16 *tail_ws = nullptr;
    f16 *qkv_res = nullptr;
    float *qkv_rbias = nullptr;
    float *attn_btab32 = nullptr;
    f16 *b96_tail = nullptr;
    float *b96_btab = nullptr;
};

struct SkipBlock {
    unsigned *list = nullptr;
    int *pixmap = nullptr;
    const nunif_swin_tail_group *groups = nullptr;
    long n_groups = 0, n_tokens = 0;
    int n_windows = 0;
};

struct SkipPlan {
    nunif_tile_grid grid = {};
    int tile_begin = 0, B = 0;
    int level = 0;
    std::vector<SkipBlock> stage[5];
    void *dev = nullptr;
    size_t bytes = 0;
    std::vector<unsigned> host;
    hipStream_t built_on = nullptr;
    hipEvent_t ready = nullptr;
};

int block_extent_back(int e, int S, int shift, int32_t *n_win, int32_t *wrap) {
    const int nw = S / 6;
    if (S <= 6) shift = 0;
    if (shift == 0) {
        *n_win = std::min(nw, (e + 5) / 6);
        *wrap = 0;
        return std::min(S, 6 * *n_win);
    }
    *n_win = std::min(nw - 1, (std::max(e - 3, 0) + 5) / 6);
    *wrap = 1;
    return *n_win == nw - 1 ? S : 3 + 6 * *n_win;
}

}
}

using namespace nunif;

extern "C" int nunif_hip_swin_unet_tile_extents(const nunif_tile_grid *g, int32_t tile_index, const int32_t *blocks_per_stage,
                                                const int32_t *shifts, int32_t to_image_fused, nunif_swin_block_extent *out) {
    (void)to_image_fused;
    NUNIF_REQUIRE(g && blocks_per_stage && shifts && out, "tile_extents: NULL argument");
    NUNIF_REQUIRE(tile_index >= 0 && tile_index < g->h_blocks * g->w_blocks, "tile_extents: tile %d outside the grid", tile_index);
    const int S = g->tile_size - 16;
    NUNIF_REQUIRE(S > 0 && S % 24 == 0 && g->scale > 0 && g->out_tile_size == S * g->scale,
                  "tile_extents: the grid is not a swin_unet grid (tile %d, output tile %d)", g->tile_size, g->out_tile_size);
    int first[6] = {0};
    for (int st = 0; st < 5; ++st) {
        NUNIF_REQUIRE(blocks_per_stage[st] >= 0, "tile_extents: negative block count");
        first[st + 1] = first[st] + blocks_per_stage[st];
    }
    const int size[5] = {S, S / 2, S / 4, S / 2, S};
    const int ti[2] = {tile_index / g->w_blocks, tile_index % g->w_blocks};
    const int y_len[2] = {g->y_h, g->y_w};
    for (int ax = 0; ax < 2; ++ax) {
        const int n_px = std::min(g->out_tile_size, y_len[ax] - g->output_tile_step * ti[ax]);
        auto stage_back = [&](int st, int e) {
            for (int i = blocks_per_stage[st] - 1; i >= 0; --i) {
                nunif_swin_block_extent &o = out[first[st] + i];
                if (e <= 0) { o.n_win[ax] = 0; o.wrap[ax] = 0; continue; }
                e = block_extent_back(e, size[st], shifts[first[st] + i], &o.n_win[ax], &o.wrap[ax]);
            }
            return std::max(e, 0);
        };
        const int e5 = n_px <= 0 ? 0 : std::min(S, (n_px + g->scale - 1) / g->scale);
        const int top_in = stage_back(4, e5);
        const int e4_in = stage_back(3, (top_in + 1) / 2);
        const int e3_in = stage_back(2, (e4_in + 1) / 2);
        const int e2_in = stage_back(1, std::min(size[1], std::max(2 * e3_in, e4_in)));
        (void)stage_back(0, std::min(size[0], std::max(2 * e2_in, top_in)));
    }
    return NUNIF_HIP_OK;
}

extern "C" int nunif_hip_swin_unet_tail_groups(const nunif_swin_block_extent *ext, int32_t n_tiles, int32_t S, int32_t shift,
                                               nunif_swin_tail_group *out, int64_t cap, int64_t *n_groups, int64_t *n_tokens) {
    const char *msg = swin_tail_groups_host(ext, n_tiles, S, shift, out, cap, n_groups, n_tokens);
    NUNIF_REQUIRE(!msg, "%s", msg);
    return NUNIF_HIP_OK;
}

struct nunif_swin_unet : DeviceOwner {
    int scale_factor = 2;
    int C = 96, heads = 6;
    int C1 = 48, C1P = 64;
    int top_dim = 96;
    float *stem1_w = nullptr, *stem1_b = nullptr;
    Linear stem2, down1, down2, up2, up1, proj2, to_image, to_image_pre;
    Linear down2b;
    bool down2_split = false;
    f16 *to_image_chained = nullptr;
    f16 *stemf_w1 = nullptr, *stemf_w2 = nullptr;
    int dir = 0;
    int att_wm = 1;
    int gelu32 = 0;
    int block96 = 0;
    bool has_proj2 = false;
    std::vector<Block> swin[5];
    DeviceBuf s1, f1, f2, f3, g1, qkv, att, hid, tile_out;
    DeviceBuf winmap[2];
    int winmap_B = 0, winmap_S = 0;
    std::list<SkipPlan> plans;
    size_t plan_bytes = 0;
    const SkipPlan *plan = nullptr;
    void drop_plan(std::list<SkipPlan>::iterator it) {
        if (it->ready) (void)hipEventDestroy(it->ready);
        (void)hipFree(it->dev);
        plan_bytes -= it->bytes;
        plans.erase(it);
    }
    void clear_plans() {
        while (!plans.empty()) drop_plan(plans.begin());
        plan = nullptr;
    }
    int device = 0;
    struct Tap { std::string name; void *dev; size_t bytes; };
    bool taps_on = false;
    std::vector<Tap> taps;
    void clear_taps() { for (auto &t : taps) (void)hipFree(t.dev); taps.clear(); }
};

namespace nunif {
namespace {

int pad16(int n) { return (n + 15) / 16 * 16; }

template <typename F>
int make_linear(nunif_swin_unet *h, int n_real, int K, F wt, const float *bias, Linear *L, bool chained = false,
                std::vector<f16> *keep = nullptr) {
    const int N = pad16(n_real);
    std::vector<f16> packed = pack_nt_ks(n_real, N, K, wt, chained);
    std::vector<float> b(N, 0.0f);
    for (int n = 0; n < n_real; ++n) b[n] = bias[n];
    L->N = N; L->n_real = n_real; L->K = K;
    if (keep) *keep = packed;
    int rc = h->upload(packed, &L->w);
    if (rc) return rc;
    return h->upload(b, &L->bias);
}

int make_plain_linear(nunif_swin_unet *h, const TensorMap &m, const std::string &key, int n_real, int K, Linear *L,
                      bool chained = false, std::vector<f16> *keep = nullptr) {
    const HostTensor *w, *b;
    int rc;
    if ((rc = find(m, key + ".weight", &w)) || (rc = find(m, key + ".bias", &b))) return rc;
    NUNIF_REQUIRE(w->numel == (int64_t)n_real * K && b->numel == n_real, "%s: unexpected shape", key.c_str());
    const float *wd = w->data;
    return make_linear(h, n_real, K, [=](int n, int k) { return wd[(size_t)n * K + k]; }, b->data, L, chained, keep);
}

int make_stage(nunif_swin_unet *h, const TensorMap &m, const std::string &key, int dim, int layers,
               std::vector<Block> *blocks) {
    blocks->resize(layers);
    const int heads = h->heads;
    for (int i = 0; i < layers; ++i) {
        const std::string p = key + ".block." + std::to_string(i) + ".";
        Block &bl = (*blocks)[i];
        int rc;
        std::vector<f16> hq;
        if ((rc = make_plain_linear(h, m, p + "attn.qkv", 3 * dim, dim, &bl.qkv, false, &hq))) return rc;
        const bool has_norm = m.find(p + "norm1.weight") != m.end();
        bl.fast = heads == 6 && (dim == 96 || dim == 192) && !has_norm;
        if (has_norm) {
            const HostTensor *n1, *n2;
            if ((rc = find(m, p + "norm1.weight", &n1)) || (rc = find(m, p + "norm2.weight", &n2))) return rc;
            NUNIF_REQUIRE(n1->numel == dim && n2->numel == dim, "%snorm: shape", p.c_str());
            NUNIF_REQUIRE(m.find(p + "norm1.bias") == m.end(), "%snorm1: LayerNorm with bias is not a reference variant", p.c_str());
            std::vector<float> g1(n1->data, n1->data + dim), g2(n2->data, n2->data + dim);
            if ((rc = h->upload(g1, &bl.norm1)) || (rc = h->upload(g2, &bl.norm2))) return rc;
        }
        if (!bl.fast) {
            if ((rc = make_plain_linear(h, m, p + "attn.proj", dim, dim, &bl.proj)) ||
                (rc = make_plain_linear(h, m, p + "mlp.0", 2 * dim, dim, &bl.mlp0p)) ||
                (rc = make_plain_linear(h, m, p + "mlp.3", dim, 2 * dim, &bl.mlp3p)))
                return rc;
        }
        if (bl.fast) {
            const HostTensor *w, *b;
            if ((rc = find(m, p + "attn.qkv.weight", &w)) || (rc = find(m, p + "attn.qkv.bias", &b))) return rc;
            const float qs = (1.0f / sqrtf((float)(dim / heads))) * 1.4426950408889634f;
            const float *wd = w->data;
            std::vector<f16> hs = pack_nt_ks(3 * dim, 3 * dim, dim, [=](int n, int k) {
                return wd[(size_t)n * dim + k] * (n < dim ? qs : 1.0f); });
            const int KS = dim / 32, NTH = (dim / heads) / 16, nf = 3 * (dim / 16) * KS;
            std::vector<f16> stream((size_t)nf * 512, (f16)0.0f);
            size_t fi = 0;
            for (int hh = 0; hh < heads; ++hh)
                for (int part = 0; part < 3; ++part)
                    for (int nt = 0; nt < NTH; ++nt)
                        for (int ks = 0; ks < KS; ++ks)
                            copy_frag(hs, (size_t)(part * (dim / 16) + hh * NTH + nt) * KS + ks, stream, &fi);
            if ((rc = h->upload(stream, &bl.qkv_res))) return rc;
            std::vector<float> rb(3 * dim);
            for (int n = 0; n < 3 * dim; ++n) rb[n] = b->data[n] * (n < dim ? qs : 1.0f);
            if ((rc = h->upload(rb, &bl.qkv_rbias))) return rc;
        }
        std::vector<f16> hp, h0, h3;
        if (bl.fast) {
        if ((rc = make_plain_linear(h, m, p + "attn.proj", dim, dim, &bl.proj, false, &hp))) return rc;
        if ((rc = make_plain_linear(h, m, p + "mlp.0", 2 * dim, dim, &bl.mlp0, true, &h0))) return rc;
        if ((rc = make_plain_linear(h, m, p + "mlp.3", dim, 2 * dim, &bl.mlp3, true, &h3))) return rc;
        }
        if (bl.fast) {
            const int KS = dim / 32, NT = dim / 16, SH = 2 * dim / 32;
            const int nf = proj_mlp_stream_frags(dim);
            std::vector<f16> stream((size_t)(nf + 15) / 16 * 16 * 512, (f16)0.0f);
            size_t fi = 0;
            auto put = [&](const std::vector<f16> &src, int frag) { copy_frag(src, frag, stream, &fi); };
            for (int sx = 0; sx < KS; ++sx)
                for (int ks = 0; ks < KS; ++ks) { put(hp, (2 * sx) * KS + ks); put(hp, (2 * sx + 1) * KS + ks); }
            for (int sx = 0; sx < SH; ++sx) {
                for (int ks = 0; ks < KS; ++ks) { put(h0, (2 * sx) * KS + ks); put(h0, (2 * sx + 1) * KS + ks); }
                for (int nt = 0; nt < NT; ++nt) put(h3, nt * SH + sx);
            }
            NUNIF_REQUIRE((int)fi == nf, "internal: tail stream has %zu fragments, expected %d", fi, nf);
            if ((rc = h->upload(stream, &bl.tail_stream))) return rc;
            if (dim == 192) {
                std::vector<f16> ws((size_t)proj_mlp_ws_stream_frags() * 512, (f16)0.0f);
                size_t wi = 0;
                auto putw = [&](const std::vector<f16> &src, int frag) { copy_frag(src, frag, ws, &wi); };
                for (int w = 0; w < 4; ++w)
                    for (int nt = 0; nt < 3; ++nt)
                        for (int ks = 0; ks < KS; ++ks) putw(hp, (3 * w + nt) * KS + ks);
                for (int w = 0; w < 4; ++w)
                    for (int nt = 0; nt < 6; ++nt)
                        for (int ks = 0; ks < KS; ++ks) putw(h0, (6 * w + nt) * KS + ks);
                for (int w = 0; w < 4; ++w)
                    for (int nt = 0; nt < 3; ++nt)
                        for (int ks = 0; ks < SH; ++ks) putw(h3, (3 * w + nt) * SH + ks);
                NUNIF_REQUIRE((int)wi == proj_mlp_ws_stream_frags(), "internal: ws tail stream has %zu fragments", wi);
                if ((rc = h->upload(ws, &bl.tail_ws))) return rc;
            }
        }
        const HostTensor *tab;
        if ((rc = find(m, p + "attn.relative_position_bias_table", &tab))) return rc;
        NUNIF_REQUIRE(tab->numel == 121 * heads, "%s: bias table shape", p.c_str());
        if (bl.fast && dim == 96) {
            const HostTensor *pw;
            if ((rc = find(m, p + "attn.proj.weight", &pw))) return rc;
            const float *pd = pw->data;
            std::vector<f16> hpc = pack_nt_ks(dim, dim, dim, [=](int n, int k) { return pd[(size_t)n * dim + k]; }, true);
            const int KS = dim / 32, NT = dim / 16, SH = 2 * dim / 32;
            std::vector<f16> stream((size_t)swin_block96_tail_frags() * 512, (f16)0.0f);
            size_t fi = 0;
            auto put = [&](const std::vector<f16> &src, int frag) { copy_frag(src, frag, stream, &fi); };
            for (int sx = 0; sx < KS; ++sx)
                for (int ks = 0; ks < KS; ++ks) { put(hpc, (2 * sx) * KS + ks); put(hpc, (2 * sx + 1) * KS + ks); }
            for (int sx = 0; sx < SH; ++sx) {
                for (int ks = 0; ks < KS; ++ks) { put(h0, (2 * sx) * KS + ks); put(h0, (2 * sx + 1) * KS + ks); }
                for (int nt = 0; nt < NT; ++nt) put(h3, nt * SH + sx);
            }
            NUNIF_REQUIRE((int)fi == swin_block96_tail_frags(), "internal: block96 stream has %zu fragments", fi);
            if ((rc = h->upload(stream, &bl.b96_tail))) return rc;
            const int stride = swin_block96_btab_floats() / heads;
            std::vector<float> rt((size_t)heads * stride, -1000.0f);
            for (int hh = 0; hh < heads; ++hh) {
                for (int i2 = 0; i2 < 121; ++i2) rt[(size_t)hh * stride + i2] = tab->data[(size_t)(120 - i2) * heads + hh] * 1.4426950408889634f;
                rt[(size_t)hh * stride + 121] = rt[(size_t)hh * stride + 122] = rt[(size_t)hh * stride + 123] = 0.0f;
            }
            if ((rc = h->upload(rt, &bl.b96_btab))) return rc;
        }
        std::vector<float> bias((size_t)heads * 36 * 48);
        for (int hh = 0; hh < heads; ++hh)
            for (int q = 0; q < 36; ++q)
                for (int k = 0; k < 48; ++k) {
                    float v = -1.0e30f;
                    if (k < 36) {
                        const int idx = (q / 6 - k / 6 + 5) * 11 + (q % 6 - k % 6 + 5);
                        v = tab->data[(size_t)idx * heads + hh];
                    }
                    bias[((size_t)hh * 36 + q) * 48 + k] = v;
                }
        if ((rc = h->upload(bias, &bl.attn_bias))) return rc;
        std::vector<float> btab32((size_t)heads * 36 * 52, 0.0f);
        for (int hh = 0; hh < heads; ++hh)
            for (int q = 0; q < 36; ++q)
                for (int k = 0; k < 48; ++k) {
                    const int key = k < 32 ? k : (((k - 32) & 3) == 0 ? 32 + ((k - 32) >> 2) : -1);
                    btab32[((size_t)hh * 36 + q) * 52 + k] =
                        key >= 0 ? bias[((size_t)hh * 36 + q) * 48 + key] * 1.4426950408889634f : -1000.0f;
                }
        if ((rc = h->upload(btab32, &bl.attn_btab32))) return rc;
    }
    return NUNIF_HIP_OK;
}

int run_gemm(const Linear &L, const f16 *a, int B, int Hi, int Wi, int Cin, int Ho, int Wo, int stride, int oy,
             int ox, int kw, int mode, int act, float slope, const f16 *res, void *out, int ldo, int ps,
             hipStream_t s, const char *tag, int rev = 0) {
    GemmArgs g;
    g.a = a; g.B = B; g.Hi = Hi; g.Wi = Wi; g.Cin = Cin;
    g.Ho = Ho; g.Wo = Wo; g.stride = stride; g.oy = oy; g.ox = ox; g.kw = kw;
    g.K = L.K; g.w = L.w; g.bias = L.bias; g.N = L.N;
    g.mode = mode; g.act = act; g.slope = slope; g.res = res; g.out = out; g.ldo = ldo;
    g.n_real = L.n_real; g.ps = ps; g.oshift = 0; g.OH = 0; g.OW = 0; g.no_clamp = 0; g.lda = 0; g.nt_chunk = 0; g.rev = rev;
    return launch_gemm(g, s, tag);
}

int run_patchup(const Linear &L, const f16 *a, int B, int H, int W, int Cq, f16 *skip, hipStream_t s, const char *tag, int rev) {
    PatchUpArgs p = {a, L.w, L.bias, skip, skip, B, H, W, Cq, rev};
    if (L.K == 192 && L.n_real == 4 * Cq && patchup_supported(p)) return launch_patchup(p, s);
    return run_gemm(L, a, B, H, W, L.K, H, W, 1, 0, 0, 1, 1, 0, 0.f, skip, skip, Cq, 1, s, tag, rev);
}

int run_patchdown(const Linear &L, const f16 *a, int B, int Ho, int Wo, int Cin, int oy, f16 *out, hipStream_t s, const char *tag,
                  int rev) {
    PatchDownArgs p;
    p.a = a; p.w = L.w; p.bias = L.bias; p.out = out; p.B = B; p.Ho = Ho; p.Wo = Wo; p.Cin = Cin; p.oy = oy; p.rev = rev;
    if (L.K == 384 && L.n_real == 192 && patchdown_supported(p)) return launch_patchdown(p, s);
    return run_gemm(L, a, B, 2 * Ho, 2 * Wo, Cin, Ho, Wo, 2, oy, 0, 2, 0, 0, 0.f, nullptr, out, L.n_real, 1, s, tag, rev);
}

int run_linear(const Linear &L, const f16 *a, int B, int H, int W, int act, const f16 *res, f16 *out,
               hipStream_t s, const char *tag, int rev = 0) {
    return run_gemm(L, a, B, H, W, L.K, H, W, 1, 0, 0, 1, 0, act, 0.f, res, out, L.n_real, 1, s, tag, rev);
}

int tap(nunif_swin_unet *h, const std::string &name, const void *src, size_t bytes, hipStream_t s) {
    if (!h->taps_on) return NUNIF_HIP_OK;
    void *p = nullptr;
    NUNIF_HIP_CHECK(hipMalloc(&p, bytes));
    NUNIF_HIP_CHECK(hipMemcpyAsync(p, src, bytes, hipMemcpyDeviceToDevice, s));
    h->taps.push_back({name, p, bytes});
    return NUNIF_HIP_OK;
}

static int next_dir(nunif_swin_unet *h) {
    const int d = h->dir;
    h->dir ^= 1;
    return d;
}

int run_stage(nunif_swin_unet *h, std::vector<Block> &blocks, f16 *x, int B, int S, int dim, hipStream_t s,
              const char *name, const TailToImage *to_image = nullptr, const std::vector<SkipBlock> *skip = nullptr) {
    f16 *qkv = (f16 *)h->qkv.p, *att = (f16 *)h->att.p;
    const size_t tok = (size_t)B * S * S;
    int rc;
    for (size_t i = 0; i < blocks.size(); ++i) {
        Block &bl = blocks[i];
        const int shift = (i % 2 == 1) ? 3 : 0;
        const std::string tn = std::string(name) + ".b" + std::to_string(i);
        if (!bl.fast) {
            f16 *hid = (f16 *)h->hid.p;
            const f16 *xin = x;
            if (bl.norm1) {
                if ((rc = launch_layernorm_nobias(x, hid, bl.norm1, (long)tok, dim, s))) return rc;
                xin = hid;
            }
            if ((rc = run_linear(bl.qkv, xin, B, S, S, 0, nullptr, qkv, s, "gemm_qkv", next_dir(h)))) return rc;
            if ((rc = tap(h, tn + ".qkv", qkv, tok * 3 * dim * 2, s))) return rc;
            if ((rc = launch_window_attn(qkv, att, bl.attn_bias, B, S, S, h->heads, dim / h->heads, shift, s))) return rc;
            if ((rc = tap(h, tn + ".attn", att, tok * dim * 2, s))) return rc;
            if ((rc = run_linear(bl.proj, att, B, S, S, 0, x, x, s, "gemm_proj", next_dir(h)))) return rc;
            xin = x;
            if (bl.norm2) {
                if ((rc = launch_layernorm_nobias(x, att, bl.norm2, (long)tok, dim, s))) return rc;
                xin = att;
            }
            if ((rc = run_linear(bl.mlp0p, xin, B, S, S, 1, nullptr, hid, s, "gemm_mlp0", next_dir(h)))) return rc;
            if ((rc = run_linear(bl.mlp3p, hid, B, S, S, 0, x, x, s, "gemm_mlp3", next_dir(h)))) return rc;
            if ((rc = tap(h, tn + ".out", x, tok * dim * 2, s))) return rc;
            continue;
        }
        const bool last_blk = i + 1 == blocks.size();
        if (dim == 96 && bl.b96_tail && h->block96 && !h->taps_on) {
            if ((rc = launch_swin_block96(x, bl.qkv_res, bl.qkv_rbias, bl.b96_btab, bl.b96_tail, bl.proj.bias, bl.mlp0.bias,
                                          bl.mlp3.bias, B, S, S, shift, s, last_blk ? to_image : nullptr, next_dir(h))))
                return rc;
            if (last_blk && to_image) break;
            continue;
        }
        const bool att_wm = dim == 96 && h->att_wm && !h->taps_on && 96L * (long)tok < (1L << 31);
        const SkipBlock *sk = skip && i < skip->size() && (*skip)[i].list && (dim == 192 ? (*skip)[i].groups != nullptr : att_wm)
                                  ? &(*skip)[i] : nullptr;
        if ((rc = launch_qkv_attn_r(x, att, bl.qkv_res, bl.qkv_rbias, bl.attn_btab32, B, S, S, dim, h->heads, shift, s, next_dir(h),
                                    att_wm ? 1 : 0, sk ? sk->list : nullptr, sk ? sk->n_windows : 0)))
            return rc;
        if ((rc = tap(h, tn + ".attn", att, tok * dim * 2, s))) return rc;
        const bool last = i + 1 == blocks.size();
        if (dim == 192) {
            if ((rc = launch_proj_mlp_ws(att, x, bl.tail_ws, bl.proj.bias, bl.mlp0.bias, bl.mlp3.bias, (long)tok, s, next_dir(h), h->gelu32,
                                         sk ? sk->groups : nullptr, sk ? sk->n_groups : 0, sk ? sk->n_tokens : 0)))
                return rc;
        } else {
            const int eff_shift = S <= 6 ? 0 : shift;
            WinMap wmap = {att_wm ? 1 : 0, S, S, eff_shift, nullptr};
            if (sk) {
                wmap.pixmap = sk->pixmap;
            } else if (att_wm) {
                if (h->winmap_S != S || B > h->winmap_B) {
                    for (int k = 0; k < 2; ++k) {
                        if ((rc = h->winmap[k].ensure(tok * sizeof(int)))) return rc;
                        if ((rc = launch_winmap_build((int *)h->winmap[k].p, B, S, S, k ? 3 : 0, s))) return rc;
                    }
                    h->winmap_B = B; h->winmap_S = S;
                }
                wmap.pixmap = (const int *)h->winmap[eff_shift ? 1 : 0].p;
            }
            if ((rc = launch_proj_mlp(att, x, bl.tail_stream, bl.proj.bias, bl.mlp0.bias, bl.mlp3.bias, sk ? 36L * sk->n_windows : (long)tok, dim, s,
                                      last ? to_image : nullptr, next_dir(h), &wmap, h->gelu32)))
                return rc;
        }
        if (last && to_image) break;
        if ((rc = tap(h, tn + ".out", x, tok * dim * 2, s))) return rc;
    }
    return NUNIF_HIP_OK;
}

int ensure_workspace(nunif_swin_unet *h, int B, int T) {
    const size_t S = T - 16, S2 = S / 2, S4 = S / 4, C = h->C;
    const size_t t1 = (size_t)B * S * S, t2 = (size_t)B * S2 * S2, t3 = (size_t)B * S4 * S4;
    const size_t top = h->top_dim;
    int rc;
    if ((rc = h->s1.ensure((size_t)B * (T - 14) * (T - 14) * h->C1P * 2))) return rc;
    if ((rc = h->f1.ensure(t1 * C * 2))) return rc;
    if ((rc = h->f2.ensure(t2 * 2 * C * 2))) return rc;
    if ((rc = h->f3.ensure(t3 * 2 * C * 2))) return rc;
    if (h->has_proj2 && (rc = h->g1.ensure(t1 * top * 2))) return rc;
    const size_t qkv_elems = std::max(t1 * 3 * std::max(C, top), t2 * 6 * C);
    if ((rc = h->qkv.ensure(qkv_elems * 2))) return rc;
    if ((rc = h->att.ensure(std::max(t1 * std::max(C, top), t2 * 2 * C) * 2))) return rc;
    if ((rc = h->hid.ensure(std::max(t1 * 2 * std::max(C, top), t2 * 4 * C) * 2))) return rc;
    return NUNIF_HIP_OK;
}

constexpr size_t kMaxPlans = 1024, kMaxPlanBytes = (size_t)1 << 30;

int skip_plan(nunif_swin_unet *h, const nunif_tile_grid *g, int t0, int B, int level, hipStream_t s, const SkipPlan **out) {
    *out = nullptr;
    const int S = g->tile_size - 16, nw = S / 6;
    if (!h->att_wm || h->taps_on || h->block96 || S <= 6 || nw >= 256 || B >= 65536 || 96L * B * S * S >= (1L << 31) ||
        g->out_tile_size != S * g->scale)
        return NUNIF_HIP_OK;
    for (auto it = h->plans.begin(); it != h->plans.end(); ++it)
        if (it->tile_begin == t0 && it->B == B && it->level == level && memcmp(g, &it->grid, sizeof(*g)) == 0) {
            h->plans.splice(h->plans.begin(), h->plans, it);
            if (it->dev && it->built_on != s) NUNIF_HIP_CHECK(hipStreamWaitEvent(s, it->ready, 0));
            *out = &*it;
            return NUNIF_HIP_OK;
        }
    int32_t per_stage[5], n_blocks = 0;
    std::vector<int32_t> shifts;
    for (int st = 0; st < 5; ++st) {
        per_stage[st] = (int32_t)h->swin[st].size();
        for (int i = 0; i < per_stage[st]; ++i) shifts.push_back(i % 2 == 1 ? 3 : 0);
        n_blocks += per_stage[st];
    }
    std::vector<std::vector<nunif_swin_block_extent>> ext(B, std::vector<nunif_swin_block_extent>(n_blocks));
    int rc;
    for (int b = 0; b < B; ++b)
        if ((rc = nunif_hip_swin_unet_tile_extents(g, t0 + b, per_stage, shifts.data(), 0, ext[b].data()))) return rc;
    h->plans.emplace_front();
    SkipPlan &plan = h->plans.front();
    auto fail = [&](int code) { h->drop_plan(h->plans.begin()); return code; };
    plan.grid = *g; plan.tile_begin = t0; plan.B = B; plan.level = level; plan.built_on = s;
    struct Piece { int st, i, shift, dim; size_t first, n, gfirst; int64_t n_groups, n_tokens; };
    std::vector<Piece> pieces;
    int first = 0;
    for (int st = 0; st < 5; first += per_stage[st], ++st) {
        const int dim = st == 0 ? h->C : (st == 4 ? h->top_dim : 2 * h->C);
        bool fast = level >= 2 ? dim == 96 || dim == 192 : (st == 0 || st == 4) && dim == 96;
        for (const Block &bl : h->swin[st]) fast = fast && bl.fast;
        if (!fast) continue;
        const int Ss = st == 0 || st == 4 ? S : (st == 2 ? S / 4 : S / 2), nw = Ss / 6;
        if (Ss <= 6) continue;
        plan.stage[st].resize(per_stage[st]);
        for (int i = 0; i < per_stage[st]; ++i) {
            const size_t at = plan.host.size();
            for (int b = 0; b < B; ++b) {
                const nunif_swin_block_extent &e = ext[b][first + i];
                auto active = [&](int ax, int w) { return w < e.n_win[ax] || (e.wrap[ax] && w == nw - 1); };
                for (int wy = 0; wy < nw; ++wy) {
                    if (!active(0, wy)) continue;
                    for (int wx = 0; wx < nw; ++wx)
                        if (active(1, wx)) plan.host.push_back((unsigned)b << 16 | (unsigned)wy << 8 | (unsigned)wx);
                }
            }
            const size_t n = plan.host.size() - at;
            if (n == (size_t)B * nw * nw || n == 0) { plan.host.resize(at); continue; }
            Piece pc = {st, i, shifts[first + i], dim, at, n, 0, 0, 0};
            if (dim == 192) {
                std::vector<nunif_swin_block_extent> eb(B);
                for (int b = 0; b < B; ++b) eb[b] = ext[b][first + i];
                const int64_t cap = (36 * (int64_t)n + 15) / 16 + 8;
                plan.host.resize((plan.host.size() + 7) / 8 * 8);
                pc.gfirst = plan.host.size();
                plan.host.resize(pc.gfirst + 8 * (size_t)cap);
                static_assert(sizeof(nunif_swin_tail_group) == 8 * sizeof(unsigned), "a group is 8 words of the plan");
                if ((rc = nunif_hip_swin_unet_tail_groups(eb.data(), B, Ss, pc.shift, (nunif_swin_tail_group *)&plan.host[pc.gfirst], cap,
                                                          &pc.n_groups, &pc.n_tokens)))
                    return fail(rc);
                plan.host.resize(pc.gfirst + 8 * (size_t)pc.n_groups);
                if (pc.n_tokens != 36 * (int64_t)n) { set_error("internal: %lld grouped tokens for %zu windows", (long long)pc.n_tokens, n); return fail(NUNIF_HIP_EINVAL); }
            }
            pieces.push_back(pc);
        }
    }
    if (pieces.empty()) { *out = &plan; return NUNIF_HIP_OK; }
    const size_t list_bytes = (plan.host.size() * 4 + 255) / 256 * 256;
    size_t n_pix = 0;
    for (const Piece &pc : pieces) n_pix += pc.dim == 96 ? pc.n * 36 : 0;
    plan.bytes = list_bytes + n_pix * 4;
    if (hipMalloc(&plan.dev, plan.bytes) != hipSuccess) {
        set_error("hipMalloc(%zu) of the window lists failed", plan.bytes);
        plan.bytes = 0;
        return fail(NUNIF_HIP_ENOMEM);
    }
    h->plan_bytes += plan.bytes;
    if (hipMemcpyAsync(plan.dev, plan.host.data(), plan.host.size() * 4, hipMemcpyHostToDevice, s) != hipSuccess ||
        hipEventCreateWithFlags(&plan.ready, hipEventDisableTiming) != hipSuccess) {
        set_error("upload of the window lists failed");
        return fail(NUNIF_HIP_EHIP);
    }
    size_t pix_at = 0;
    for (const Piece &pc : pieces) {
        SkipBlock &sb = plan.stage[pc.st][pc.i];
        sb.list = (unsigned *)plan.dev + pc.first;
        sb.n_windows = (int)pc.n;
        if (pc.dim == 192) {
            sb.groups = (const nunif_swin_tail_group *)((unsigned *)plan.dev + pc.gfirst);
            sb.n_groups = (long)pc.n_groups; sb.n_tokens = (long)pc.n_tokens;
            continue;
        }
        sb.pixmap = (int *)((char *)plan.dev + list_bytes) + pix_at;
        pix_at += pc.n * 36;
        if ((rc = launch_winmap_list_build(sb.pixmap, sb.list, sb.n_windows, S, S, pc.shift, s))) return fail(rc);
    }
    if (hipEventRecord(plan.ready, s) != hipSuccess) { set_error("hipEventRecord failed"); return fail(NUNIF_HIP_EHIP); }
    while (h->plans.size() > kMaxPlans || (h->plan_bytes > kMaxPlanBytes && h->plans.size() > 1)) h->drop_plan(std::prev(h->plans.end()));
    *out = &plan;
    return NUNIF_HIP_OK;
}

int forward_impl(nunif_swin_unet *h, const float *x, const float *frame, const nunif_tile_grid *grid,
                 int tile_begin, float *z, int B, int T, hipStream_t s, int skip_pad = 0) {
    const int S = T - 16, C = h->C;
    NUNIF_REQUIRE(T > 16 && S % 12 == 0 && S % 16 == 0, "tile_size %d is not valid for swin_unet", T);
    int rc;
    if ((rc = ensure_workspace(h, B, T))) return rc;
    h->plan = nullptr;
    if (frame && skip_pad && (rc = skip_plan(h, grid, tile_begin, B, skip_pad, s, &h->plan))) return rc;
    auto skip_of = [&](int st) { return h->plan && !h->plan->stage[st].empty() ? &h->plan->stage[st] : nullptr; };
    f16 *s1 = (f16 *)h->s1.p, *f1 = (f16 *)h->f1.p, *f2 = (f16 *)h->f2.p, *f3 = (f16 *)h->f3.p;

    if (h->stemf_w2 && stem_fused_supported(h->C1, (int)C)) {
        StemFusedArgs sf;
        memset(&sf, 0, sizeof(sf));
        if (frame) {
            sf.x = frame; sf.frame_mode = 1; sf.H = grid->x_h; sf.W = grid->x_w; sf.wb = grid->w_blocks;
            sf.istep = grid->input_tile_step; sf.pad_t = grid->pad_t; sf.pad_l = grid->pad_l; sf.tile_begin = tile_begin;
        } else {
            sf.x = x;
        }
        sf.B = B; sf.T = T; sf.w1 = h->stemf_w1; sf.w2 = h->stemf_w2; sf.b2 = h->stem2.bias; sf.out = f1; sf.slope = 0.1f;
        h->dir = 1;
        if ((rc = launch_stem_fused(sf, s))) return rc;
        goto stem_done;
    }
    Stem1Args a1;
    memset(&a1, 0, sizeof(a1));
    if (frame) {
        a1.x = frame; a1.frame_mode = 1; a1.H = grid->x_h; a1.W = grid->x_w; a1.wb = grid->w_blocks;
        a1.istep = grid->input_tile_step; a1.pad_t = grid->pad_t; a1.pad_l = grid->pad_l; a1.tile_begin = tile_begin;
    } else {
        a1.x = x;
    }
    a1.B = B; a1.T = T; a1.w = h->stem1_w; a1.bias = h->stem1_b; a1.C1 = h->C1; a1.C1P = h->C1P; a1.out = s1;
    a1.slope = 0.1f;
    h->dir = 1;
    if ((rc = launch_stem1(a1, s))) return rc;
    if ((rc = run_gemm(h->stem2, s1, B, T - 14, T - 14, h->C1P, S, S, 1, 0, 0, 3, 0, 2, 0.1f, nullptr, f1, C, 1, s,
                              "gemm_stem2", next_dir(h))))
        return rc;
stem_done:
    if ((rc = tap(h, "stem", f1, (size_t)B * S * S * C * 2, s))) return rc;
    if ((rc = run_stage(h, h->swin[0], f1, B, S, C, s, "swin1", nullptr, skip_of(0)))) return rc;
    if ((rc = run_patchdown(h->down1, f1, B, S / 2, S / 2, C, 0, f2, s, "gemm_down1", next_dir(h)))) return rc;
    if ((rc = tap(h, "down1", f2, (size_t)B * (S / 2) * (S / 2) * 2 * C * 2, s))) return rc;
    if ((rc = run_stage(h, h->swin[1], f2, B, S / 2, 2 * C, s, "swin2", nullptr, skip_of(1)))) return rc;
    if (h->down2_split) {
        if ((rc = run_patchdown(h->down2, f2, B, S / 4, S / 4, 2 * C, 0, f3, s, "gemm_down2", next_dir(h)))) return rc;
    } else if ((rc = run_gemm(h->down2, f2, B, S / 2, S / 2, 2 * C, S / 4, S / 4, 2, 0, 0, 2, 0, 0, 0.f, nullptr, f3,
                              2 * C, 1, s, "gemm_down2", next_dir(h))))
        return rc;
    if (h->down2_split && (rc = run_gemm(h->down2b, f2, B, S / 2, S / 2, 2 * C, S / 4, S / 4, 2, 1, 0, 2, 0, 0, 0.f, f3, f3,
                                         2 * C, 1, s, "gemm_down2b", next_dir(h))))
        return rc;
    if ((rc = tap(h, "down2", f3, (size_t)B * (S / 4) * (S / 4) * 2 * C * 2, s))) return rc;
    if ((rc = run_stage(h, h->swin[2], f3, B, S / 4, 2 * C, s, "swin3", nullptr, skip_of(2)))) return rc;
    if ((rc = run_patchup(h->up2, f3, B, S / 4, S / 4, 2 * C, f2, s, "gemm_up2", next_dir(h)))) return rc;
    if ((rc = tap(h, "up2", f2, (size_t)B * (S / 2) * (S / 2) * 2 * C * 2, s))) return rc;
    if ((rc = run_stage(h, h->swin[3], f2, B, S / 2, 2 * C, s, "swin4", nullptr, skip_of(3)))) return rc;
    f16 *top = f1;
    if (h->has_proj2) {
        top = (f16 *)h->g1.p;
        if ((rc = run_linear(h->proj2, f1, B, S, S, 0, nullptr, top, s, "gemm_proj2", next_dir(h)))) return rc;
    }
    if ((rc = run_patchup(h->up1, f2, B, S / 2, S / 2, h->top_dim, top, s, "gemm_up1", next_dir(h)))) return rc;
    if ((rc = tap(h, "up1", top, (size_t)B * S * S * h->top_dim * 2, s))) return rc;
    if (h->top_dim == 96 && h->swin[4].back().fast && h->to_image_chained && !h->taps_on) {
        TailToImage ti;
        ti.w = h->to_image_chained; ti.bias = h->to_image.bias; ti.out = z; ti.H = S; ti.W = S; ti.ps = h->scale_factor;
        ti.n_real = h->to_image.n_real;
        return run_stage(h, h->swin[4], top, B, S, h->top_dim, s, "swin5", &ti, skip_of(4));
    }
    if ((rc = run_stage(h, h->swin[4], top, B, S, h->top_dim, s, "swin5", nullptr, skip_of(4)))) return rc;
    if (h->scale_factor == 8) {
        f16 *pre = (f16 *)h->att.p;
        if ((rc = run_gemm(h->to_image_pre, top, B, S, S, h->top_dim, S, S, 1, 0, 0, 1, 0, 2, 0.2f, nullptr, pre, 192, 1, s,
                           "gemm_to_image_pre", next_dir(h))))
            return rc;
        top = pre;
    }
    if ((rc = run_gemm(h->to_image, top, B, S, S, h->top_dim, S, S, 1, 0, 0, 1, 2, 0, 0.f, nullptr, z, 0,
                       h->scale_factor, s, "gemm_to_image", next_dir(h))))
        return rc;
    return NUNIF_HIP_OK;
}

}
}

extern "C" int nunif_hip_swin_unet_create(const nunif_tensor_desc *tensors, int32_t n_tensors,
                                          int32_t scale_factor, nunif_swin_unet **handle) {
    NUNIF_REQUIRE(tensors && handle && n_tensors > 0, "swin_unet_create: NULL argument");
    NUNIF_REQUIRE(scale_factor == 1 || scale_factor == 2 || scale_factor == 4 || scale_factor == 8,
                  "swin_unet_create: scale_factor %d unsupported (1, 2, 4, 8)", scale_factor);
    const TensorMap m = tensor_map(tensors, n_tensors);
    nunif_swin_unet *h = new nunif_swin_unet();
    (void)hipGetDevice(&h->device);
    if (const char *v = getenv("NUNIF_BLOCK96")) h->block96 = atoi(v);
    if (const char *v = getenv("NUNIF_ATT_WM")) h->att_wm = atoi(v);
    h->gelu32 = scale_factor == 1;
    if (const char *v = getenv("NUNIF_SWIN_GELU32")) h->gelu32 = atoi(v);
    h->scale_factor = scale_factor;
    const std::string P = "unet.";
    int rc = NUNIF_HIP_OK;
    do {
        const HostTensor *w0, *b0, *w2, *b2;
        if ((rc = find(m, P + "patch.0.weight", &w0)) || (rc = find(m, P + "patch.0.bias", &b0)) ||
            (rc = find(m, P + "patch.2.weight", &w2)) || (rc = find(m, P + "patch.2.bias", &b2)))
            break;
        if (w2->shape.size() != 4 || w0->shape.size() != 4 || w0->shape[1] != 3) {
            set_error("patch conv: unexpected shape"); rc = NUNIF_HIP_EINVAL; break;
        }
        const int C = (int)w2->shape[0];
        const int C1 = (int)w0->shape[0];
        if (C % 96 != 0 || C1 * 2 != C) { set_error("base_dim %d unsupported", C); rc = NUNIF_HIP_EUNSUPPORTED; break; }
        h->C = C; h->heads = C / 16; h->C1 = C1; h->C1P = (C1 + 31) / 32 * 32;
        h->has_proj2 = scale_factor >= 4;
        h->top_dim = h->has_proj2 ? 2 * C : C;
        {
            std::vector<float> w(w0->data, w0->data + w0->numel), b(b0->data, b0->data + b0->numel);
            if ((rc = h->upload(w, &h->stem1_w)) || (rc = h->upload(b, &h->stem1_b))) break;
        }
        {
            const float *wd = w2->data;
            const int C1P = h->C1P;
            rc = make_linear(h, C, 9 * C1P, [=](int n, int k) {
                const int tap = k / C1P, ci = k % C1P;
                return ci < C1 ? wd[((size_t)n * C1 + ci) * 9 + tap] : 0.0f;
            }, b2->data, &h->stem2);
            if (rc) break;
        }
        if (stem_fused_supported(C1, C)) {
            const float *w0d = w0->data, *b0d = b0->data, *wd = w2->data;
            std::vector<f16> p1 = pack_nt_ks(C1, pad16(C1), 32, [=](int n, int k) {
                return k < 27 ? w0d[(size_t)n * 27 + k] : (k == 27 ? b0d[n] : 0.0f); });
            const int K2 = 448;
            std::vector<f16> stream = pack_ks_nt(C, C, K2, [=](int n, int k) {
                const int tap = k / C1, ci = k % C1;
                return k < 9 * C1 ? wd[((size_t)n * C1 + ci) * 9 + tap] : 0.0f; }, false, 0);
            if ((rc = h->upload(p1, &h->stemf_w1)) || (rc = h->upload(stream, &h->stemf_w2))) break;
        }
        if ((rc = make_stage(h, m, P + "swin1", C, 2, &h->swin[0]))) break;
        if ((rc = make_stage(h, m, P + "swin2", 2 * C, 2, &h->swin[1]))) break;
        if ((rc = make_stage(h, m, P + "swin3", 2 * C, 6, &h->swin[2]))) break;
        if ((rc = make_stage(h, m, P + "swin4", 2 * C, 2, &h->swin[3]))) break;
        if ((rc = make_stage(h, m, P + "swin5", h->top_dim, 2, &h->swin[4]))) break;
        auto make_down = [&](const std::string &key, int cin, int cout, Linear *L) -> int {
            const HostTensor *w, *b;
            int r;
            if ((r = find(m, key + ".conv.weight", &w)) || (r = find(m, key + ".conv.bias", &b))) return r;
            NUNIF_REQUIRE(w->numel == (int64_t)cout * cin * 4, "%s: shape", key.c_str());
            const float *wd = w->data;
            return make_linear(h, cout, 4 * cin, [=](int n, int k) {
                const int tap = k / cin, ci = k % cin;
                return wd[((size_t)n * cin + ci) * 4 + tap];
            }, b->data, L);
        };
        auto make_up = [&](const std::string &key, int cin, int cq, Linear *L) -> int {
            const HostTensor *w, *b;
            int r;
            if ((r = find(m, key + ".proj.weight", &w)) || (r = find(m, key + ".proj.bias", &b))) return r;
            NUNIF_REQUIRE(w->numel == (int64_t)4 * cq * cin, "%s: shape", key.c_str());
            const float *wd = w->data;
            std::vector<float> bb(4 * cq);
            for (int n = 0; n < 4 * cq; ++n) bb[n] = b->data[(n % cq) * 4 + n / cq];
            return make_linear(h, 4 * cq, cin, [=](int n, int k) {
                const int q = n / cq, c = n % cq;
                return wd[((size_t)(c * 4 + q)) * cin + k];
            }, bb.data(), L);
        };
        if ((rc = make_down(P + "down1", C, 2 * C, &h->down1))) break;
        {
            const HostTensor *w, *b;
            if ((rc = find(m, P + "down2.conv.weight", &w)) || (rc = find(m, P + "down2.conv.bias", &b))) break;
            const int cin = 2 * C, cout = 2 * C;
            if (w->numel != (int64_t)cout * cin * 4) { set_error("down2: shape"); rc = NUNIF_HIP_EINVAL; break; }
            const float *wd = w->data;
            std::vector<float> zero(cout, 0.0f);
            if ((rc = make_linear(h, cout, 2 * cin, [=](int n, int k) {
                    const int dx = k / cin, ci = k % cin; return wd[((size_t)n * cin + ci) * 4 + dx]; }, b->data, &h->down2)) ||
                (rc = make_linear(h, cout, 2 * cin, [=](int n, int k) {
                    const int dx = k / cin, ci = k % cin; return wd[((size_t)n * cin + ci) * 4 + 2 + dx]; }, zero.data(), &h->down2b)))
                break;
            h->down2_split = true;
        }
        if ((rc = make_up(P + "up2", 2 * C, 2 * C, &h->up2))) break;
        if ((rc = make_up(P + "up1", 2 * C, h->top_dim, &h->up1))) break;
        if (h->has_proj2 && (rc = make_plain_linear(h, m, P + "proj2", 2 * C, C, &h->proj2))) break;
        if (scale_factor == 8) {
            if ((rc = make_plain_linear(h, m, P + "to_image.proj.0", 192, h->top_dim, &h->to_image_pre)) ||
                (rc = make_plain_linear(h, m, P + "to_image.proj.2", 192, 192, &h->to_image)))
                break;
        } else if ((rc = make_plain_linear(h, m, P + "to_image.proj", 3 * scale_factor * scale_factor, h->top_dim,
                                           &h->to_image)))
            break;
        if (h->top_dim == 96 && 3 * scale_factor * scale_factor <= 16) {
            const HostTensor *tw;
            if ((rc = find(m, P + "to_image.proj.weight", &tw))) break;
            const float *wd = tw->data;
            const int nr = 3 * scale_factor * scale_factor, K = h->top_dim;
            std::vector<f16> ch = pack_nt_ks(nr, pad16(nr), K, [=](int n, int k) { return wd[(size_t)n * K + k]; }, true);
            if ((rc = h->upload(ch, &h->to_image_chained))) break;
        }
    } while (0);
    if (rc) {
        nunif_hip_swin_unet_destroy(h);
        return rc;
    }
    *handle = h;
    return NUNIF_HIP_OK;
}

extern "C" int nunif_hip_swin_unet_debug_taps(nunif_swin_unet *h, int32_t enable) {
    NUNIF_REQUIRE(h, "debug_taps: NULL handle");
    h->clear_taps();
    h->taps_on = enable != 0;
    return NUNIF_HIP_OK;
}

extern "C" int nunif_hip_swin_unet_get_tap(nunif_swin_unet *h, int32_t index, char *name, int32_t name_cap,
                                           void *host_dst, int64_t cap_bytes, int64_t *nbytes) {
    NUNIF_REQUIRE(h && nbytes, "get_tap: NULL argument");
    if (index < 0 || index >= (int)h->taps.size()) return 1;
    const auto &t = h->taps[index];
    if (name && name_cap > 0) { strncpy(name, t.name.c_str(), name_cap - 1); name[name_cap - 1] = 0; }
    *nbytes = (int64_t)t.bytes;
    if (host_dst) {
        NUNIF_REQUIRE(cap_bytes >= (int64_t)t.bytes, "get_tap: buffer too small");
        NUNIF_HIP_CHECK(hipDeviceSynchronize());
        NUNIF_HIP_CHECK(hipMemcpy(host_dst, t.dev, t.bytes, hipMemcpyDeviceToHost));
    }
    return NUNIF_HIP_OK;
}

extern "C" void nunif_hip_swin_unet_destroy(nunif_swin_unet *h) {
    if (!h) return;
    h->clear_taps();
    h->clear_plans();
    h->free_all();
    for (DeviceBuf *b : {&h->s1, &h->f1, &h->f2, &h->f3, &h->g1, &h->qkv, &h->att, &h->hid, &h->tile_out, &h->winmap[0], &h->winmap[1]}) b->release();
    delete h;
}

extern "C" int nunif_hip_swin_unet_forward(nunif_swin_unet *h, const float *x, float *z, int32_t batch,
                                           int32_t tile_size, void *stream) {
    NUNIF_REQUIRE(h && x && z && batch > 0, "swin_unet_forward: bad argument");
    return forward_impl(h, x, nullptr, nullptr, 0, z, batch, tile_size, (hipStream_t)stream);
}

static int skip_pad_level() {
    const char *v = getenv("NUNIF_SWIN_SKIP_PAD");
    if (!v) return 2;
    const int l = atoi(v);
    return l <= 0 ? 0 : (l == 1 ? 1 : 2);
}

extern "C" int nunif_hip_swin_unet_tail192_test(nunif_swin_unet *h, int32_t stage, int32_t block, const void *att, void *x,
                                                int64_t n_tokens, const nunif_swin_tail_group *groups, int64_t n_groups,
                                                int64_t n_listed, int32_t rev, void *stream) {
    NUNIF_REQUIRE(h && att && x && n_tokens > 0 && stage >= 0 && stage < 5 && block >= 0 && block < (int)h->swin[stage].size(),
                  "tail192_test: bad argument");
    const Block &bl = h->swin[stage][block];
    NUNIF_REQUIRE(bl.fast && bl.tail_ws, "tail192_test: stage %d block %d has no C = 192 tail", stage, block);
    return launch_proj_mlp_ws((const f16 *)att, (f16 *)x, bl.tail_ws, bl.proj.bias, bl.mlp0.bias, bl.mlp3.bias, (long)n_tokens,
                              (hipStream_t)stream, rev ? 1 : 0, h->gelu32, groups, (long)n_groups, (long)n_listed);
}

extern "C" int nunif_hip_swin_unet_render(nunif_swin_unet *h, const float *x, float *y, int32_t x_h, int32_t x_w,
                                          int32_t tile_size, int32_t batch_size, void *stream) {
    NUNIF_REQUIRE(h && x && y && batch_size > 0, "swin_unet_render: bad argument");
    NUNIF_REQUIRE(h->scale_factor != 8, "swin_unet_render: the 8x net has no consistent tile geometry; use forward");
    const int s = h->scale_factor;
    nunif_tile_grid g;
    int rc = nunif_hip_tile_grid_init(x_h, x_w, s, 8 * s, tile_size, 4 * s, &g);
    if (rc) return rc;
    const int n_tiles = g.h_blocks * g.w_blocks;
    const size_t To = g.out_tile_size;
    if ((rc = h->tile_out.ensure((size_t)n_tiles * 3 * To * To * sizeof(float)))) return rc;
    float *tile_out = (float *)h->tile_out.p;
    hipStream_t st = (hipStream_t)stream;
    const int skip_pad = skip_pad_level();
    for (int t0 = 0; t0 < n_tiles; t0 += batch_size) {
        const int nb = std::min(batch_size, n_tiles - t0);
        if ((rc = forward_impl(h, nullptr, x, &g, t0, tile_out + (size_t)t0 * 3 * To * To, nb, tile_size, st, skip_pad)))
            return rc;
    }
    return launch_stitch(tile_out, y, &g, 3, st);
}

static int rows_grid(nunif_swin_unet *h, int32_t x_h, int32_t x_w, int32_t tile_size, nunif_tile_grid *g) {
    NUNIF_REQUIRE(h->scale_factor != 8, "swin_unet: the 8x net has no consistent tile geometry");
    const int s = h->scale_factor;
    int rc = nunif_hip_tile_grid_init(x_h, x_w, s, 8 * s, tile_size, 4 * s, g);
    if (rc) return rc;
    const size_t To = g->out_tile_size;
    return h->tile_out.ensure((size_t)g->h_blocks * g->w_blocks * 3 * To * To * sizeof(float));
}

extern "C" int nunif_hip_swin_unet_render_tile_rows(nunif_swin_unet *h, const float *x, int32_t x_h, int32_t x_w,
                                                    int32_t tile_size, int32_t batch_size, int32_t row_begin,
                                                    int32_t row_end, void *stream) {
    NUNIF_REQUIRE(h && x && batch_size > 0, "swin_unet_render_tile_rows: bad argument");
    nunif_tile_grid g;
    int rc = rows_grid(h, x_h, x_w, tile_size, &g);
    if (rc) return rc;
    NUNIF_REQUIRE(0 <= row_begin && row_begin <= row_end && row_end <= g.h_blocks, "tile rows [%d, %d) outside the grid of %d rows",
                  row_begin, row_end, g.h_blocks);
    const size_t To = g.out_tile_size;
    float *tile_out = (float *)h->tile_out.p;
    const int t_end = row_end * g.w_blocks;
    const int skip_pad = skip_pad_level();
    for (int t0 = row_begin * g.w_blocks; t0 < t_end; t0 += batch_size) {
        const int nb = std::min(batch_size, t_end - t0);
        if ((rc = forward_impl(h, nullptr, x, &g, t0, tile_out + (size_t)t0 * 3 * To * To, nb, tile_size, (hipStream_t)stream, skip_pad)))
            return rc;
    }
    return NUNIF_HIP_OK;
}

extern "C" int nunif_hip_swin_unet_tile_row_band(nunif_swin_unet *h, int32_t x_h, int32_t x_w, int32_t tile_size,
                                                 int32_t tile_row, int32_t row0, int32_t n_rows, float *band,
                                                 int32_t import_band, void *stream) {
    NUNIF_REQUIRE(h && band, "swin_unet_tile_row_band: bad argument");
    nunif_tile_grid g;
    int rc = rows_grid(h, x_h, x_w, tile_size, &g);
    if (rc) return rc;
    const int To = g.out_tile_size;
    NUNIF_REQUIRE(0 <= tile_row && tile_row < g.h_blocks && row0 >= 0 && n_rows > 0 && row0 + n_rows <= To, "tile_row_band: bad window");
    float *store = (float *)h->tile_out.p + (size_t)tile_row * g.w_blocks * 3 * To * To + (size_t)row0 * To;
    const size_t planes = (size_t)g.w_blocks * 3;
    if (import_band)
        NUNIF_HIP_CHECK(hipMemcpy2DAsync(store, (size_t)To * To * 4, band, (size_t)n_rows * To * 4, (size_t)n_rows * To * 4, planes,
                                         hipMemcpyDeviceToDevice, (hipStream_t)stream));
    else
        NUNIF_HIP_CHECK(hipMemcpy2DAsync(band, (size_t)n_rows * To * 4, store, (size_t)To * To * 4, (size_t)n_rows * To * 4, planes,
                                         hipMemcpyDeviceToDevice, (hipStream_t)stream));
    return NUNIF_HIP_OK;
}

extern "C" int nunif_hip_swin_unet_stitch_rows(nunif_swin_unet *h, float *y_band, int32_t x_h, int32_t x_w, int32_t tile_size,
                                               int32_t y_row_begin, int32_t y_row_end, void *stream) {
    NUNIF_REQUIRE(h && y_band, "swin_unet_stitch_rows: bad argument");
    nunif_tile_grid g;
    int rc = rows_grid(h, x_h, x_w, tile_size, &g);
    if (rc) return rc;
    return launch_stitch((const float *)h->tile_out.p, y_band, &g, 3, (hipStream_t)stream, y_row_begin, y_row_end - y_row_begin, 1);
}
```

Baseline: 340.6 MPix/s.

## Restrict patch up/down producers to tokens needed by listed swin windows

```diff
diff --git a/include/nunif_hip.h b/include/nunif_hip.h
--- a/include/nunif_hip.h
+++ b/include/nunif_hip.h
@@ -83,6 +83,15 @@
 } nunif_swin_tail_group;
 int nunif_hip_swin_unet_tail_groups(const nunif_swin_block_extent *ext, int32_t n_tiles, int32_t S, int32_t shift,
                                     nunif_swin_tail_group *out, int64_t cap, int64_t *n_groups, int64_t *n_tokens);
+
+enum { NUNIF_SWIN_PRODUCER_STEM = 0, NUNIF_SWIN_PRODUCER_DOWN1 = 1, NUNIF_SWIN_PRODUCER_DOWN2 = 2, NUNIF_SWIN_PRODUCER_UP2 = 3,
+       NUNIF_SWIN_PRODUCER_UP1 = 4 };
+int nunif_hip_swin_unet_producer_tokens(const nunif_swin_block_extent *ext, int32_t n_tiles, const int32_t *blocks_per_stage,
+                                        const int32_t *shifts, const int32_t *listed, int32_t S, int32_t f1_whole, int32_t producer,
+                                        int32_t patch_h, int32_t patch_w, uint32_t *out, int64_t cap, int64_t *n_out);
+
+int nunif_hip_swin_unet_down2_test(nunif_swin_unet *handle, const void *a, void *out, int32_t B, int32_t Ho, int32_t Wo,
+                                   int32_t acc_form, void *stream);
 
 int nunif_hip_swin_unet_tail192_test(nunif_swin_unet *handle, int32_t stage, int32_t block, const void *att, void *x,
                                      int64_t n_tokens, const nunif_swin_tail_group *groups, int64_t n_groups, int64_t n_listed,
diff --git a/nunif_amd/_hip.py b/nunif_amd/_hip.py
--- a/nunif_amd/_hip.py
+++ b/nunif_amd/_hip.py
@@ -86,6 +86,10 @@
                                                    c_int32, ctypes.POINTER(SwinBlockExtent)]),
     "nunif_hip_swin_unet_tail_groups": (c_int32, [ctypes.POINTER(SwinBlockExtent), c_int32, c_int32, c_int32,
                                                   ctypes.POINTER(SwinTailGroup), c_int64, ctypes.POINTER(c_int64), ctypes.POINTER(c_int64)]),
+    "nunif_hip_swin_unet_producer_tokens": (c_int32, [ctypes.POINTER(SwinBlockExtent), c_int32, ctypes.POINTER(c_int32), ctypes.POINTER(c_int32),
+                                                      ctypes.POINTER(c_int32), c_int32, c_int32, c_int32, c_int32, c_int32,
+                                                      ctypes.POINTER(ctypes.c_uint32), c_int64, ctypes.POINTER(c_int64)]),
+    "nunif_hip_swin_unet_down2_test": (c_int32, [c_void_p, c_void_p, c_void_p, c_int32, c_int32, c_int32, c_int32, c_void_p]),
     "nunif_hip_swin_unet_tail192_test": (c_int32, [c_void_p, c_int32, c_int32, c_void_p, c_void_p, c_int64, c_void_p, c_int64, c_int64,
                                                    c_int32, c_void_p]),
     "nunif_hip_swin_unet_v2_create": (c_int32, [ctypes.POINTER(TensorDesc), c_int32, c_int32, ctypes.POINTER(c_void_p)]),
@@ -316,6 +320,32 @@
     return (SwinTailGroup * ng.value).from_buffer(out) if ng.value else (SwinTailGroup * 0)(), nt.value
 
 
+SWIN_PRODUCERS = {"stem": 0, "down1": 1, "down2": 2, "up2": 3, "up1": 4}
+
+
+def swin_producer_tokens(extents, S, producer, blocks_per_stage=(2, 2, 6, 2, 2), shifts=None, listed=None, f1_whole=False,
+                         patch=(24, 16)):
+    n_blocks = sum(blocks_per_stage)
+    if shifts is None:
+        shifts = [3 if i % 2 else 0 for k in blocks_per_stage for i in range(k)]
+    ext = (SwinBlockExtent * (len(extents) * n_blocks))()
+    for t, tile in enumerate(extents):
+        assert len(tile) == n_blocks
+        for i, (ny, nx, wy, wx) in enumerate(tile):
+            e = ext[t * n_blocks + i]
+            e.n_win[0], e.n_win[1], e.wrap[0], e.wrap[1] = ny, nx, wy, wx
+    per = (c_int32 * 5)(*blocks_per_stage)
+    sh = (c_int32 * n_blocks)(*shifts)
+    li = (c_int32 * n_blocks)(*[1 if v else 0 for v in listed]) if listed is not None else None
+    args = (ext, len(extents), per, sh, li, S, 1 if f1_whole else 0, SWIN_PRODUCERS[producer], patch[0], patch[1])
+    n = c_int64(0)
+    check(lib().nunif_hip_swin_unet_producer_tokens(*args, None, 0, ctypes.byref(n)))
+    cap = (n.value + 31) // 32 * 32
+    out = (ctypes.c_uint32 * max(1, cap))()
+    check(lib().nunif_hip_swin_unet_producer_tokens(*args, out, cap, ctypes.byref(n)))
+    return list(out)[:n.value if producer == "stem" else cap], n.value
+
+
 def blend_ramp(blend_size):
     buf = (c_float * max(1, blend_size))()
     check(lib().nunif_hip_blend_ramp(blend_size, buf))
diff --git a/nunif_amd/csrc/swin_kernels.h b/nunif_amd/csrc/swin_kernels.h
--- a/nunif_amd/csrc/swin_kernels.h
+++ b/nunif_amd/csrc/swin_kernels.h
@@ -28,12 +28,15 @@
 };
 int launch_gemm(const GemmArgs &g, hipStream_t s, const char *tag);
 
-struct PatchUpArgs { const f16 *a, *w; const float *bias; const f16 *res; f16 *out; int B, Ho, Wo, Cq, rev; };
+struct PatchUpArgs { const f16 *a, *w; const float *bias; const f16 *res; f16 *out; int B, Ho, Wo, Cq, rev;
+                     const unsigned *list = nullptr; unsigned n_list = 0; };
 bool patchup_supported(const PatchUpArgs &g);
 int launch_patchup(const PatchUpArgs &g, hipStream_t s);
 
-struct PatchDownArgs { const f16 *a, *w; const float *bias; f16 *out; int B, Ho, Wo, Cin, oy, rev; int N = 192; int act = 0; float slope = 0.f; };
+struct PatchDownArgs { const f16 *a, *w; const float *bias; f16 *out; int B, Ho, Wo, Cin, oy, rev; int N = 192; int act = 0; float slope = 0.f;
+                       const unsigned *list = nullptr; unsigned n_list = 0; int acc = 0; };
 bool patchdown_supported(const PatchDownArgs &g);
+bool patchdown_acc_enabled();
 int launch_patchdown(const PatchDownArgs &g, hipStream_t s);
 
 struct CunetUpArgs { const f16 *a, *w; const float *bias; const f16 *res; f16 *out; const float *in_scale; int B, S, res_S, crop;
diff --git a/nunif_amd/csrc/swin_patchdown.hip b/nunif_amd/csrc/swin_patchdown.hip
--- a/nunif_amd/csrc/swin_patchdown.hip
+++ b/nunif_amd/csrc/swin_patchdown.hip
@@ -10,7 +10,7 @@
 constexpr int kMF = 2;
 }
 
-template <int CIN, int kKS, int kNT, bool LRELU>
+template <int CIN, int kKS, int kNT, bool LRELU, bool LISTED = false, bool ACC = false>
 __global__ void __launch_bounds__(kWaves * 64) patchdown_kernel(PatchDownArgs g) {
     static_assert(CIN == 64 || CIN == 96 || CIN == 192, "Cin");
     constexpr int kWBytes = kNT * kKS * 1024;
@@ -30,7 +30,7 @@
         if (tid < kNT * 4) reinterpret_cast<float4 *>(smem_pd + kWBytes)[tid] = reinterpret_cast<const float4 *>(g.bias)[tid];
     }
     const unsigned Wo = (unsigned)g.Wo, Ho = (unsigned)g.Ho, Wi = 2 * Wo, Hi = 2 * Ho;
-    const unsigned M = (unsigned)g.B * Ho * Wo;
+    const unsigned M = LISTED ? g.n_list : (unsigned)g.B * Ho * Wo;
     const unsigned n_groups = (M + kMF * 16 - 1) / (kMF * 16);
     const unsigned step = gridDim.x * kWaves;
     unsigned gi = blockIdx.x * kWaves + wave;
@@ -38,12 +38,23 @@
     const int prc = pair_run_channel(grp);
 
     struct Grp { unsigned in[kMF], out[kMF]; };
-    auto coords = [&](unsigned gidx, Grp &c) {
+    struct Tok { unsigned m[kMF]; };
+    auto fetch_tok = [&](unsigned gidx, Tok &t) {
         const unsigned gg = g.rev ? n_groups - 1 - gidx : gidx;
 #pragma unroll
+        for (int f = 0; f < kMF; ++f) t.m[f] = g.list[gg * (kMF * 16) + f * 16 + r16];
+    };
+    auto coords = [&](unsigned gidx, const Tok &tk, Grp &c) {
+        const unsigned gg = g.rev ? n_groups - 1 - gidx : gidx;
+#pragma unroll
         for (int f = 0; f < kMF; ++f) {
-            unsigned m = gg * (kMF * 16) + f * 16 + r16;
-            m = m < M ? m : M - 1;
+            unsigned m;
+            if constexpr (LISTED) {
+                m = tk.m[f];
+            } else {
+                m = gg * (kMF * 16) + f * 16 + r16;
+                m = m < M ? m : M - 1;
+            }
             const unsigned t = m / Wo, x = m - t * Wo;
             const unsigned b = t / Ho, y = t - b * Ho;
             c.in[f] = (((b * Hi + 2 * y + (unsigned)g.oy) * Wi + 2 * x) * CIN + grp * 8) * 2;
@@ -61,8 +72,15 @@
     };
 
     Grp cur, nxt;
+    Tok tnx = {};
     f16x8 xf[kMF][kKS];
-    coords(any ? gi : 0, cur);
+    if constexpr (LISTED) {
+        fetch_tok(any ? gi : 0, tnx);
+        coords(any ? gi : 0, tnx, cur);
+        fetch_tok(gi + step < n_groups ? gi + step : (any ? gi : 0), tnx);
+    } else {
+        coords(any ? gi : 0, tnx, cur);
+    }
 #pragma unroll
     for (int ks = 0; ks < kKS; ++ks) {
 #pragma unroll
@@ -73,6 +91,10 @@
     for (int ks = 0; ks < kKS; ++ks) {
 #pragma unroll
         for (int f = 0; f < kMF; ++f) asm volatile("" : "+v"(xf[f][ks]));
+    }
+    if constexpr (LISTED) {
+#pragma unroll
+        for (int f = 0; f < kMF; ++f) asm volatile("" : "+v"(tnx.m[f]));
     }
     __syncthreads();
     if (!any) return;
@@ -80,15 +102,31 @@
     while (true) {
         const unsigned gn = gi + step;
         const bool has_next = gn < n_groups;
-        coords(has_next ? gn : gi, nxt);
+        coords(has_next ? gn : gi, tnx, nxt);
+        if constexpr (LISTED) {
+            const unsigned g2 = gn + step;
+            fetch_tok(g2 < n_groups ? g2 : gi, tnx);
+        }
         int lofs = lane;
         asm volatile("" : "+v"(lofs));
         f32x4 acc[kNT][kMF];
+        constexpr int kResLead = ACC ? kNT / 4 : 0;
+        f16x8 rres[ACC ? kNT / 2 : 1][kMF];
+        auto load_res = [&](int p) {
+#pragma unroll
+            for (int f = 0; f < kMF; ++f)
+                rres[p][f] = *reinterpret_cast<const f16x8 *>(reinterpret_cast<const unsigned char *>(g.out) + (size_t)cur.out[f] + p * 64);
+        };
 #pragma unroll
         for (int nt = 0; nt < kNT; ++nt) {
-            const float4 bv = bres[nt * 4 + (lofs >> 4)];
-#pragma unroll
-            for (int f = 0; f < kMF; ++f) acc[nt][f] = (f32x4){bv.x, bv.y, bv.z, bv.w};
+            if constexpr (ACC) {
+#pragma unroll
+                for (int f = 0; f < kMF; ++f) acc[nt][f] = (f32x4){0.f, 0.f, 0.f, 0.f};
+            } else {
+                const float4 bv = bres[nt * 4 + (lofs >> 4)];
+#pragma unroll
+                for (int f = 0; f < kMF; ++f) acc[nt][f] = (f32x4){bv.x, bv.y, bv.z, bv.w};
+            }
         }
 #pragma unroll
         for (int ks = 0; ks < kKS; ++ks) {
@@ -100,6 +138,12 @@
             }
 #pragma unroll
             for (int f = 0; f < kMF; ++f) xf[f][ks] = load_frag(nxt, f, ks);
+            if constexpr (ACC) {
+                if (ks == kKS - 4) {
+#pragma unroll
+                    for (int p = 0; p < kResLead; ++p) load_res(p);
+                }
+            }
             __builtin_amdgcn_sched_barrier(0);
         }
         unsigned char *obase = reinterpret_cast<unsigned char *>(g.out);
@@ -108,6 +152,15 @@
 #pragma unroll
             for (int f = 0; f < kMF; ++f) {
                 f32x4 a0 = acc[2 * p][f], a1 = acc[2 * p + 1][f];
+                if constexpr (ACC) {
+                    const float4 b0 = bres[(2 * p) * 4 + (lofs >> 4)], b1 = bres[(2 * p + 1) * 4 + (lofs >> 4)];
+                    f16x4 ra, rb;
+                    run_to_pair(rres[p][f], ra, rb);
+                    a0 = (f32x4){a0[0] + b0.x, a0[1] + b0.y, a0[2] + b0.z, a0[3] + b0.w};
+                    a1 = (f32x4){a1[0] + b1.x, a1[1] + b1.y, a1[2] + b1.z, a1[3] + b1.w};
+#pragma unroll
+                    for (int r = 0; r < 4; ++r) { a0[r] += (float)ra[r]; a1[r] += (float)rb[r]; }
+                }
                 if constexpr (LRELU) {
 #pragma unroll
                     for (int r = 0; r < 4; ++r) {
@@ -119,11 +172,19 @@
                                              (f16x4){(f16)a1[0], (f16)a1[1], (f16)a1[2], (f16)a1[3]});
                 *reinterpret_cast<f16x8 *>(obase + (size_t)cur.out[f] + p * 64) = ov;
             }
+            if constexpr (ACC) {
+                if (p + kResLead < kNT / 2) load_res(p + kResLead);
+            }
         }
         if (!has_next) break;
         cur = nxt;
         gi = gn;
     }
+}
+
+bool patchdown_acc_enabled() {
+    const char *e = getenv("NUNIF_PATCHDOWN_ACC");
+    return !(e && atoi(e) == 0);
 }
 
 bool patchdown_supported(const PatchDownArgs &g) {
@@ -132,18 +193,20 @@
     const bool shape = (g.Cin == 96 && g.N == 192 && g.oy == 0) || (g.Cin == 192 && g.N == 192 && (g.oy == 0 || g.oy == 1)) ||
                        (g.Cin == 64 && g.N == 64 && g.oy == 0);
     const bool act_ok = g.Cin == 64 ? g.act == 2 : g.act == 0;
-    return shape && M > 0 && 4 * M * g.Cin * 2 < (1L << 32) && M * g.N * 2 < (1L << 32) && act_ok;
-}
-
-template <int CIN, int KS, int NT, bool LRELU>
+    const bool list_ok = !g.list || (g.Cin == 192 && g.n_list > 0 && (long)g.n_list <= M);
+    const bool acc_ok = !g.acc || (g.Cin == 192 && patchdown_acc_enabled());
+    return shape && M > 0 && 4 * M * g.Cin * 2 < (1L << 32) && M * g.N * 2 < (1L << 32) && act_ok && list_ok && acc_ok;
+}
+
+template <int CIN, int KS, int NT, bool LRELU, bool LISTED = false, bool ACC = false>
 static int launch_pd(const PatchDownArgs &g, hipStream_t s, const char *name, int wgs_per_cu) {
     constexpr int smem = NT * KS * 1024 + NT * 16 * 4;
     static_assert(smem <= 160 * 1024, "LDS");
-    const long M = (long)g.B * g.Ho * g.Wo;
+    const long M = LISTED ? (long)g.n_list : (long)g.B * g.Ho * g.Wo;
     static bool configured = false;
     static int cus = 256;
     if (!configured) {
-        NUNIF_HIP_CHECK(hipFuncSetAttribute((const void *)patchdown_kernel<CIN, KS, NT, LRELU>, hipFuncAttributeMaxDynamicSharedMemorySize, smem));
+        NUNIF_HIP_CHECK(hipFuncSetAttribute((const void *)patchdown_kernel<CIN, KS, NT, LRELU, LISTED, ACC>, hipFuncAttributeMaxDynamicSharedMemorySize, smem));
         int dev = 0;
         NUNIF_HIP_CHECK(hipGetDevice(&dev));
         NUNIF_HIP_CHECK(hipDeviceGetAttribute(&cus, hipDeviceAttributeMultiprocessorCount, dev));
@@ -151,8 +214,8 @@
     }
     const long groups = (M + kMF * 16 - 1) / (kMF * 16);
     const unsigned grid = (unsigned)std::max<long>(1, std::min<long>((groups + kWaves - 1) / kWaves, (long)cus * wgs_per_cu));
-    ProfScope ps(name, s, 2.0 * (double)M * (KS * 32.0) * (NT * 16.0), (double)M * (KS * 32.0 + NT * 16.0) * 2.0);
-    patchdown_kernel<CIN, KS, NT, LRELU><<<grid, kWaves * 64, smem, s>>>(g);
+    ProfScope ps(name, s, 2.0 * (double)M * (KS * 32.0) * (NT * 16.0), (double)M * (KS * 32.0 + NT * 16.0 * (ACC ? 2.0 : 1.0)) * 2.0);
+    patchdown_kernel<CIN, KS, NT, LRELU, LISTED, ACC><<<grid, kWaves * 64, smem, s>>>(g);
     NUNIF_LAUNCH_CHECK();
     return NUNIF_HIP_OK;
 }
@@ -160,7 +223,12 @@
 int launch_patchdown(const PatchDownArgs &g, hipStream_t s) {
     NUNIF_REQUIRE(g.a && g.w && g.bias && g.out && patchdown_supported(g), "patchdown: bad argument");
     if (g.Cin == 96) return launch_pd<96, 12, 12, false>(g, s, "patchdown_kernel<96>", 1);
-    if (g.Cin == 192) return launch_pd<192, 12, 12, false>(g, s, "patchdown_kernel<192>", 1);
+    if (g.Cin == 192 && g.acc)
+        return g.list ? launch_pd<192, 12, 12, false, true, true>(g, s, "patchdown_kernel<192,listed,acc>", 1)
+                      : launch_pd<192, 12, 12, false, false, true>(g, s, "patchdown_kernel<192,acc>", 1);
+    if (g.Cin == 192)
+        return g.list ? launch_pd<192, 12, 12, false, true>(g, s, "patchdown_kernel<192,listed>", 1)
+                      : launch_pd<192, 12, 12, false>(g, s, "patchdown_kernel<192>", 1);
     return launch_pd<64, 8, 4, true>(g, s, "patchdown_kernel<64>", 2);
 }
 
diff --git a/nunif_amd/csrc/swin_patchup.hip b/nunif_amd/csrc/swin_patchup.hip
--- a/nunif_amd/csrc/swin_patchup.hip
+++ b/nunif_amd/csrc/swin_patchup.hip
@@ -21,7 +21,7 @@
 static_assert(kTrips % kD == 0, "the ring slot of a trip is static");
 }
 
-template <int CQ>
+template <int CQ, bool LISTED = false>
 __global__ void __launch_bounds__(kWaves * 64) patchup_kernel(PatchUpArgs g) {
     constexpr int HALVES = 4 * CQ / (kNT * 16);
     static_assert(HALVES == 1 || HALVES == 2, "Cq is 96 or 192");
@@ -45,7 +45,7 @@
     }
 
     const unsigned Wo = (unsigned)g.Wo, Ho = (unsigned)g.Ho;
-    const unsigned M = (unsigned)g.B * Ho * Wo;
+    const unsigned M = LISTED ? g.n_list : (unsigned)g.B * Ho * Wo;
     const unsigned n_groups = (M + kMF * 16 - 1) / (kMF * 16);
     const unsigned step = nwb * kWaves;
     unsigned gi = wb * kWaves + wave;
@@ -58,12 +58,23 @@
         return (unsigned)(((q >> 1) * 2 * Wo + (q & 1)) * CQ + c);
     };
     struct Grp { unsigned pix[kMF], xo[kMF]; };
-    auto coords = [&](unsigned gidx, Grp &c) {
+    struct Tok { unsigned m[kMF]; };
+    auto fetch_tok = [&](unsigned gidx, Tok &t) {
         const unsigned gg = g.rev ? n_groups - 1 - gidx : gidx;
 #pragma unroll
+        for (int f = 0; f < kMF; ++f) t.m[f] = g.list[gg * (kMF * 16) + f * 16 + r16];
+    };
+    auto coords = [&](unsigned gidx, const Tok &tk, Grp &c) {
+        const unsigned gg = g.rev ? n_groups - 1 - gidx : gidx;
+#pragma unroll
         for (int f = 0; f < kMF; ++f) {
-            unsigned m = gg * (kMF * 16) + f * 16 + r16;
-            m = m < M ? m : M - 1;
+            unsigned m;
+            if constexpr (LISTED) {
+                m = tk.m[f];
+            } else {
+                m = gg * (kMF * 16) + f * 16 + r16;
+                m = m < M ? m : M - 1;
+            }
             const unsigned t = m / Wo, x = m - t * Wo;
             const unsigned b = t / Ho, y = t - b * Ho;
             c.xo[f] = (m * (kKS * 32) + grp * 8) * 2;
@@ -87,7 +98,14 @@
     Grp cur, nxt;
     f16x8 xc[kMF][kKS], xn[kMF][kKS];
     f16x8 rr[kD][kMF];
-    coords(any ? gi : 0, cur);
+    Tok tnx = {};
+    if constexpr (LISTED) {
+        fetch_tok(any ? gi : 0, tnx);
+        coords(any ? gi : 0, tnx, cur);
+        fetch_tok(gi + step < n_groups ? gi + step : (any ? gi : 0), tnx);
+    } else {
+        coords(any ? gi : 0, tnx, cur);
+    }
     load_x(cur, xc);
 #pragma unroll
     for (int t = 0; t < kD; ++t) load_res(cur, t, rr[t]);
@@ -98,6 +116,7 @@
         for (int ks = 0; ks < kKS; ++ks) asm volatile("" : "+v"(xc[f][ks]));
 #pragma unroll
         for (int t = 0; t < kD; ++t) asm volatile("" : "+v"(rr[t][f]));
+        if constexpr (LISTED) asm volatile("" : "+v"(tnx.m[f]));
     }
     __syncthreads();
     if (!any) return;
@@ -105,7 +124,11 @@
     while (true) {
         const unsigned gn = gi + step;
         const bool has_next = gn < n_groups;
-        coords(has_next ? gn : gi, nxt);
+        coords(has_next ? gn : gi, tnx, nxt);
+        if constexpr (LISTED) {
+            const unsigned g2 = gn + step;
+            fetch_tok(g2 < n_groups ? g2 : gi, tnx);
+        }
         load_x(nxt, xn);
         int lofs = lane;
         asm volatile("" : "+v"(lofs));
@@ -175,17 +198,20 @@
 bool patchup_supported(const PatchUpArgs &g) {
     if (const char *e = getenv("NUNIF_PATCHUP")) if (atoi(e) == 0) return false;
     const long M = (long)g.B * g.Ho * g.Wo;
-    return (g.Cq == 96 || g.Cq == 192) && g.res && M > 0 && M * 384 < (1L << 32) && M * 8 * g.Cq < (1L << 32);
+    const bool list_ok = !g.list || (g.n_list > 0 && (long)g.n_list <= M);
+    return (g.Cq == 96 || g.Cq == 192) && g.res && M > 0 && M * 384 < (1L << 32) && M * 8 * g.Cq < (1L << 32) && list_ok;
 }
 
 int launch_patchup(const PatchUpArgs &g, hipStream_t s) {
     NUNIF_REQUIRE(g.a && g.w && g.bias && g.res && g.out && patchup_supported(g), "patchup: bad argument");
-    const long M = (long)g.B * g.Ho * g.Wo;
+    const long M = g.list ? (long)g.n_list : (long)g.B * g.Ho * g.Wo;
     static bool configured = false;
     static int cus = 256;
     if (!configured) {
         NUNIF_HIP_CHECK(hipFuncSetAttribute((const void *)patchup_kernel<96>, hipFuncAttributeMaxDynamicSharedMemorySize, kSmem));
         NUNIF_HIP_CHECK(hipFuncSetAttribute((const void *)patchup_kernel<192>, hipFuncAttributeMaxDynamicSharedMemorySize, kSmem));
+        NUNIF_HIP_CHECK(hipFuncSetAttribute((const void *)patchup_kernel<96, true>, hipFuncAttributeMaxDynamicSharedMemorySize, kSmem));
+        NUNIF_HIP_CHECK(hipFuncSetAttribute((const void *)patchup_kernel<192, true>, hipFuncAttributeMaxDynamicSharedMemorySize, kSmem));
         int dev = 0;
         NUNIF_HIP_CHECK(hipGetDevice(&dev));
         NUNIF_HIP_CHECK(hipDeviceGetAttribute(&cus, hipDeviceAttributeMultiprocessorCount, dev));
@@ -197,7 +223,13 @@
     const unsigned grid = (unsigned)(per_half * halves);
     const double flops = 2.0 * (double)M * 192.0 * 4.0 * g.Cq;
     const double bytes = (double)M * (192.0 * 2.0 + 4.0 * g.Cq * 2.0 * 2.0);
-    if (g.Cq == 96) {
+    if (g.list && g.Cq == 96) {
+        ProfScope ps("patchup_kernel<96,listed>", s, flops, bytes);
+        patchup_kernel<96, true><<<grid, kWaves * 64, kSmem, s>>>(g);
+    } else if (g.list) {
+        ProfScope ps("patchup_kernel<192,listed>", s, flops, bytes);
+        patchup_kernel<192, true><<<grid, kWaves * 64, kSmem, s>>>(g);
+    } else if (g.Cq == 96) {
         ProfScope ps("patchup_kernel<96>", s, flops, bytes);
         patchup_kernel<96><<<grid, kWaves * 64, kSmem, s>>>(g);
     } else {
diff --git a/nunif_amd/csrc/swin_producer_tokens_host.h b/nunif_amd/csrc/swin_producer_tokens_host.h
--- /dev/null
+++ b/nunif_amd/csrc/swin_producer_tokens_host.h
@@ -0,0 +1,128 @@
+#pragma once
+#include <cstdint>
+#include <vector>
+
+#include "../../include/nunif_hip.h"
+
+namespace nunif {
+
+inline const char *swin_producer_tokens_host(const nunif_swin_block_extent *ext, int32_t n_tiles, const int32_t *blocks_per_stage,
+                                             const int32_t *shifts, const int32_t *listed, int32_t S, int32_t f1_whole,
+                                             int32_t producer, int32_t patch_h, int32_t patch_w, uint32_t *out, int64_t cap,
+                                             int64_t *n_out) {
+    if (!(ext && blocks_per_stage && shifts && n_out && n_tiles > 0)) return "producer_tokens: bad argument";
+    if (!(S >= 24 && S % 24 == 0 && (int64_t)n_tiles * S * S < ((int64_t)1 << 31))) return "producer_tokens: tile count or side unsupported";
+    if (producer < NUNIF_SWIN_PRODUCER_STEM || producer > NUNIF_SWIN_PRODUCER_UP1) return "producer_tokens: unknown producer";
+    if (producer == NUNIF_SWIN_PRODUCER_STEM && (patch_h <= 0 || patch_w <= 0)) return "producer_tokens: the stem needs its patch size";
+    int first[6] = {0};
+    for (int st = 0; st < 5; ++st) {
+        if (blocks_per_stage[st] < 1) return "producer_tokens: a stage without blocks";
+        first[st + 1] = first[st] + blocks_per_stage[st];
+    }
+    const int n_blocks = first[5];
+    const int size[5] = {S, S / 2, S / 4, S / 2, S};
+    for (int i = 0; i < n_blocks; ++i)
+        if (shifts[i] != 0 && shifts[i] != 3) return "producer_tokens: shift unsupported";
+    typedef std::vector<char> Set;
+    auto parents = [](const Set &a) { Set p(a.size() / 2); for (size_t i = 0; i < p.size(); ++i) p[i] = a[2 * i] | a[2 * i + 1]; return p; };
+    auto children = [](const Set &a) { Set c(a.size() * 2); for (size_t i = 0; i < c.size(); ++i) c[i] = a[i / 2]; return c; };
+    auto join = [](Set &a, const Set &b) { for (size_t i = 0; i < a.size(); ++i) a[i] |= b[i]; };
+    int64_t n = 0;
+    auto put = [&](uint32_t v) -> bool {
+        if (out) {
+            if (n >= cap) return false;
+            out[n] = v;
+        }
+        ++n;
+        return true;
+    };
+    Set want[2];
+    std::vector<int> ys, runs;
+    for (int b = 0; b < n_tiles; ++b) {
+        bool same = b > 0;
+        for (int i = 0; same && i < n_blocks; ++i) {
+            const nunif_swin_block_extent &p = ext[(size_t)(b - 1) * n_blocks + i], &q = ext[(size_t)b * n_blocks + i];
+            same = p.n_win[0] == q.n_win[0] && p.n_win[1] == q.n_win[1] && p.wrap[0] == q.wrap[0] && p.wrap[1] == q.wrap[1];
+        }
+        for (int ax = 0; ax < 2 && !same; ++ax) {
+            Set R[5];
+            for (int st = 0; st < 5; ++st) {
+                const int Ss = size[st], nw = Ss / 6;
+                R[st].assign(Ss, 0);
+                for (int i = first[st]; i < first[st + 1]; ++i) {
+                    if (listed && !listed[i]) { R[st].assign(Ss, 1); break; }
+                    const nunif_swin_block_extent &e = ext[(size_t)b * n_blocks + i];
+                    if (e.n_win[ax] < 0 || e.n_win[ax] > nw) return "producer_tokens: more windows than the side holds";
+                    const int shift = Ss <= 6 ? 0 : shifts[i];
+                    for (int w = 0; w < nw; ++w) {
+                        if (!(w < e.n_win[ax] || (e.wrap[ax] && w == nw - 1))) continue;
+                        for (int t = 0; t < 6; ++t) R[st][(6 * w + shift + t) % Ss] = 1;
+                    }
+                }
+            }
+            const Set up1 = parents(R[4]), up2 = parents(R[3]);
+            Set n3 = R[2];
+            join(n3, up2);
+            Set n2 = R[1];
+            join(n2, children(n3));
+            join(n2, up1);
+            Set n1 = R[0];
+            join(n1, children(n2));
+            if (f1_whole) n1.assign(S, 1);
+            switch (producer) {
+                case NUNIF_SWIN_PRODUCER_STEM: want[ax] = n1; break;
+                case NUNIF_SWIN_PRODUCER_DOWN1: want[ax] = n2; break;
+                case NUNIF_SWIN_PRODUCER_DOWN2: want[ax] = n3; break;
+                case NUNIF_SWIN_PRODUCER_UP2: want[ax] = up2; break;
+                default: want[ax] = up1; break;
+            }
+        }
+        if (producer == NUNIF_SWIN_PRODUCER_STEM) {
+            const int nty = (S + patch_h - 1) / patch_h, ntx = (S + patch_w - 1) / patch_w;
+            Set py(nty, 0), px(ntx, 0);
+            for (int y = 0; y < S; ++y) py[y / patch_h] |= want[0][y];
+            for (int x = 0; x < S; ++x) px[x / patch_w] |= want[1][x];
+            for (int ty = 0; ty < nty; ++ty)
+                for (int tx = 0; tx < ntx; ++tx)
+                    if (py[ty] && px[tx] && !put((uint32_t)((b * nty + ty) * ntx + tx))) return "producer_tokens: the table is too small";
+            continue;
+        }
+        const int Ss = (int)want[0].size();
+        if (!same) {
+            ys.clear(); runs.clear();
+            for (int y = 0; y < Ss; ++y)
+                if (want[0][y]) ys.push_back(y);
+            for (int x = 0; x < Ss;) {
+                if (!want[1][x]) { ++x; continue; }
+                int x1 = x;
+                while (x1 < Ss && want[1][x1]) ++x1;
+                runs.push_back(x); runs.push_back(x1);
+                x = x1;
+            }
+        }
+        int per_row = 0;
+        for (size_t k = 0; k < runs.size(); k += 2) per_row += runs[k + 1] - runs[k];
+        const int64_t add = (int64_t)ys.size() * per_row;
+        if (out) {
+            if (n + add > cap) return "producer_tokens: the table is too small";
+            uint32_t *o = out + n;
+            for (int y : ys) {
+                const uint32_t row = (uint32_t)((b * Ss + y) * Ss);
+                for (size_t k = 0; k < runs.size(); k += 2)
+                    for (int x = runs[k]; x < runs[k + 1]; ++x) *o++ = row + (uint32_t)x;
+            }
+        }
+        n += add;
+    }
+    *n_out = n;
+    if (producer != NUNIF_SWIN_PRODUCER_STEM && out && n > 0) {
+        const uint32_t last = out[n - 1];
+        for (int64_t i = n; i < (n + 31) / 32 * 32; ++i) {
+            if (i >= cap) return "producer_tokens: the table is too small";
+            out[i] = last;
+        }
+    }
+    return nullptr;
+}
+
+}
diff --git a/nunif_amd/csrc/swin_unet.cpp b/nunif_amd/csrc/swin_unet.cpp
--- a/nunif_amd/csrc/swin_unet.cpp
+++ b/nunif_amd/csrc/swin_unet.cpp
@@ -8,6 +8,7 @@
 
 #include "host_weights.h"
 #include "swin_kernels.h"
+#include "swin_producer_tokens_host.h"
 #include "swin_tail_groups_host.h"
 
 namespace nunif {
@@ -46,11 +47,18 @@
     int n_windows = 0;
 };
 
+struct ProducerList {
+    const unsigned *list = nullptr;
+    unsigned n = 0;
+};
+
 struct SkipPlan {
     nunif_tile_grid grid = {};
     int tile_begin = 0, B = 0;
     int level = 0;
     std::vector<SkipBlock> stage[5];
+    ProducerList producer[5];
+    bool producers = false;
     void *dev = nullptr;
     size_t bytes = 0;
     std::vector<unsigned> host;
@@ -109,6 +117,16 @@
         const int e2_in = stage_back(1, std::min(size[1], std::max(2 * e3_in, e4_in)));
         (void)stage_back(0, std::min(size[0], std::max(2 * e2_in, top_in)));
     }
+    return NUNIF_HIP_OK;
+}
+
+extern "C" int nunif_hip_swin_unet_producer_tokens(const nunif_swin_block_extent *ext, int32_t n_tiles, const int32_t *blocks_per_stage,
+                                                   const int32_t *shifts, const int32_t *listed, int32_t S, int32_t f1_whole,
+                                                   int32_t producer, int32_t patch_h, int32_t patch_w, uint32_t *out, int64_t cap,
+                                                   int64_t *n_out) {
+    const char *msg = swin_producer_tokens_host(ext, n_tiles, blocks_per_stage, shifts, listed, S, f1_whole, producer, patch_h, patch_w,
+                                                out, cap, n_out);
+    NUNIF_REQUIRE(!msg, "%s", msg);
     return NUNIF_HIP_OK;
 }
 
@@ -336,17 +354,23 @@
     return launch_gemm(g, s, tag);
 }
 
-int run_patchup(const Linear &L, const f16 *a, int B, int H, int W, int Cq, f16 *skip, hipStream_t s, const char *tag, int rev) {
+int run_patchup(const Linear &L, const f16 *a, int B, int H, int W, int Cq, f16 *skip, hipStream_t s, const char *tag, int rev,
+                const ProducerList *pl = nullptr) {
     PatchUpArgs p = {a, L.w, L.bias, skip, skip, B, H, W, Cq, rev};
+    if (pl && pl->list) { p.list = pl->list; p.n_list = pl->n; }
     if (L.K == 192 && L.n_real == 4 * Cq && patchup_supported(p)) return launch_patchup(p, s);
+    NUNIF_REQUIRE(!p.list, "%s: no listed form of this PatchUp", tag);
     return run_gemm(L, a, B, H, W, L.K, H, W, 1, 0, 0, 1, 1, 0, 0.f, skip, skip, Cq, 1, s, tag, rev);
 }
 
 int run_patchdown(const Linear &L, const f16 *a, int B, int Ho, int Wo, int Cin, int oy, f16 *out, hipStream_t s, const char *tag,
-                  int rev) {
+                  int rev, const ProducerList *pl = nullptr, int acc = 0) {
     PatchDownArgs p;
-    p.a = a; p.w = L.w; p.bias = L.bias; p.out = out; p.B = B; p.Ho = Ho; p.Wo = Wo; p.Cin = Cin; p.oy = oy; p.rev = rev;
+    p.a = a; p.w = L.w; p.bias = L.bias; p.out = out; p.B = B; p.Ho = Ho; p.Wo = Wo; p.Cin = Cin; p.oy = oy; p.rev = rev; p.acc = acc;
+    if (pl && pl->list) { p.list = pl->list; p.n_list = pl->n; }
     if (L.K == 384 && L.n_real == 192 && patchdown_supported(p)) return launch_patchdown(p, s);
+    NUNIF_REQUIRE(!p.list, "%s: no listed form of this PatchDown", tag);
+    if (acc) return run_gemm(L, a, B, 2 * Ho, 2 * Wo, Cin, Ho, Wo, 2, oy, 0, 2, 0, 0, 0.f, out, out, L.n_real, 1, s, tag, rev);
     return run_gemm(L, a, B, 2 * Ho, 2 * Wo, Cin, Ho, Wo, 2, oy, 0, 2, 0, 0, 0.f, nullptr, out, L.n_real, 1, s, tag, rev);
 }
 
@@ -485,10 +509,11 @@
         for (int i = 0; i < per_stage[st]; ++i) shifts.push_back(i % 2 == 1 ? 3 : 0);
         n_blocks += per_stage[st];
     }
-    std::vector<std::vector<nunif_swin_block_extent>> ext(B, std::vector<nunif_swin_block_extent>(n_blocks));
+    std::vector<nunif_swin_block_extent> ext((size_t)B * n_blocks);
+    std::vector<int32_t> listed(n_blocks, 0);
     int rc;
     for (int b = 0; b < B; ++b)
-        if ((rc = nunif_hip_swin_unet_tile_extents(g, t0 + b, per_stage, shifts.data(), 0, ext[b].data()))) return rc;
+        if ((rc = nunif_hip_swin_unet_tile_extents(g, t0 + b, per_stage, shifts.data(), 0, &ext[(size_t)b * n_blocks]))) return rc;
     h->plans.emplace_front();
     SkipPlan &plan = h->plans.front();
     auto fail = [&](int code) { h->drop_plan(h->plans.begin()); return code; };
@@ -507,7 +532,7 @@
         for (int i = 0; i < per_stage[st]; ++i) {
             const size_t at = plan.host.size();
             for (int b = 0; b < B; ++b) {
-                const nunif_swin_block_extent &e = ext[b][first + i];
+                const nunif_swin_block_extent &e = ext[(size_t)b * n_blocks + first + i];
                 auto active = [&](int ax, int w) { return w < e.n_win[ax] || (e.wrap[ax] && w == nw - 1); };
                 for (int wy = 0; wy < nw; ++wy) {
                     if (!active(0, wy)) continue;
@@ -520,7 +545,7 @@
             Piece pc = {st, i, shifts[first + i], dim, at, n, 0, 0, 0};
             if (dim == 192) {
                 std::vector<nunif_swin_block_extent> eb(B);
-                for (int b = 0; b < B; ++b) eb[b] = ext[b][first + i];
+                for (int b = 0; b < B; ++b) eb[b] = ext[(size_t)b * n_blocks + first + i];
                 const int64_t cap = (36 * (int64_t)n + 15) / 16 + 8;
                 plan.host.resize((plan.host.size() + 7) / 8 * 8);
                 pc.gfirst = plan.host.size();
@@ -533,9 +558,33 @@
                 if (pc.n_tokens != 36 * (int64_t)n) { set_error("internal: %lld grouped tokens for %zu windows", (long long)pc.n_tokens, n); return fail(NUNIF_HIP_EINVAL); }
             }
             pieces.push_back(pc);
+            listed[first + i] = 1;
         }
     }
     if (pieces.empty()) { *out = &plan; return NUNIF_HIP_OK; }
+    struct ProdPiece { int producer; size_t first; int64_t n; };
+    std::vector<ProdPiece> prods;
+    if (level >= 3 && h->C == 96 && h->down2_split && S % 24 == 0) {
+        for (int pr = NUNIF_SWIN_PRODUCER_DOWN2; pr <= NUNIF_SWIN_PRODUCER_UP1; ++pr) {
+            const int Sp = pr == NUNIF_SWIN_PRODUCER_UP1 ? S / 2 : S / 4;
+            const int64_t whole = (int64_t)B * Sp * Sp;
+            int64_t n = 0;
+            if ((rc = nunif_hip_swin_unet_producer_tokens(ext.data(), B, per_stage, shifts.data(), listed.data(), S, h->has_proj2 ? 1 : 0, pr, 0,
+                                                          0, nullptr, 0, &n)))
+                return fail(rc);
+            if (n <= 0 || n > whole) { set_error("internal: producer %d lists %lld of %lld", pr, (long long)n, (long long)whole); return fail(NUNIF_HIP_EINVAL); }
+            if (n == whole) continue;
+            const int64_t cap = (n + 31) / 32 * 32;
+            plan.host.resize((plan.host.size() + 7) / 8 * 8);
+            const size_t at = plan.host.size();
+            plan.host.resize(at + (size_t)cap);
+            if ((rc = nunif_hip_swin_unet_producer_tokens(ext.data(), B, per_stage, shifts.data(), listed.data(), S, h->has_proj2 ? 1 : 0, pr, 0,
+                                                          0, &plan.host[at], cap, &n)))
+                return fail(rc);
+            prods.push_back({pr, at, n});
+        }
+        plan.producers = true;
+    }
     const size_t list_bytes = (plan.host.size() * 4 + 255) / 256 * 256;
     size_t n_pix = 0;
     for (const Piece &pc : pieces) n_pix += pc.dim == 96 ? pc.n * 36 : 0;
@@ -564,6 +613,10 @@
         sb.pixmap = (int *)((char *)plan.dev + list_bytes) + pix_at;
         pix_at += pc.n * 36;
         if ((rc = launch_winmap_list_build(sb.pixmap, sb.list, sb.n_windows, S, S, pc.shift, s))) return fail(rc);
+    }
+    for (const ProdPiece &pp : prods) {
+        plan.producer[pp.producer].list = (const unsigned *)plan.dev + pp.first;
+        plan.producer[pp.producer].n = (unsigned)pp.n;
     }
     if (hipEventRecord(plan.ready, s) != hipSuccess) { set_error("hipEventRecord failed"); return fail(NUNIF_HIP_EHIP); }
     while (h->plans.size() > kMaxPlans || (h->plan_bytes > kMaxPlanBytes && h->plans.size() > 1)) h->drop_plan(std::prev(h->plans.end()));
@@ -581,6 +634,15 @@
     if (frame && skip_pad && (rc = skip_plan(h, grid, tile_begin, B, skip_pad, s, &h->plan))) return rc;
     auto skip_of = [&](int st) { return h->plan && !h->plan->stage[st].empty() ? &h->plan->stage[st] : nullptr; };
     f16 *s1 = (f16 *)h->s1.p, *f1 = (f16 *)h->f1.p, *f2 = (f16 *)h->f2.p, *f3 = (f16 *)h->f3.p;
+    bool lp = h->plan && h->plan->producers;
+    if (lp) {
+        PatchDownArgs d1, d2;
+        d1.B = B; d1.Ho = d1.Wo = S / 4; d1.Cin = 2 * (int)C; d1.oy = 0; d1.rev = 0;
+        d2 = d1; d2.oy = 1; d2.acc = 1;
+        PatchUpArgs u2 = {f3, nullptr, nullptr, f2, f2, B, S / 4, S / 4, 2 * (int)C, 0}, u1 = {f2, nullptr, nullptr, f1, f1, B, S / 2, S / 2, h->top_dim, 0};
+        lp = patchdown_supported(d1) && patchdown_supported(d2) && patchup_supported(u2) && patchup_supported(u1);
+    }
+    auto prod_of = [&](int pr) { return lp ? &h->plan->producer[pr] : nullptr; };
 
     if (h->stemf_w2 && stem_fused_supported(h->C1, (int)C)) {
         StemFusedArgs sf;
@@ -614,20 +676,20 @@
 stem_done:
     if ((rc = tap(h, "stem", f1, (size_t)B * S * S * C * 2, s))) return rc;
     if ((rc = run_stage(h, h->swin[0], f1, B, S, C, s, "swin1", nullptr, skip_of(0)))) return rc;
-    if ((rc = run_patchdown(h->down1, f1, B, S / 2, S / 2, C, 0, f2, s, "gemm_down1", next_dir(h)))) return rc;
+    if ((rc = run_patchdown(h->down1, f1, B, S / 2, S / 2, C, 0, f2, s, "gemm_down1", next_dir(h), prod_of(NUNIF_SWIN_PRODUCER_DOWN1)))) return rc;
     if ((rc = tap(h, "down1", f2, (size_t)B * (S / 2) * (S / 2) * 2 * C * 2, s))) return rc;
     if ((rc = run_stage(h, h->swin[1], f2, B, S / 2, 2 * C, s, "swin2", nullptr, skip_of(1)))) return rc;
     if (h->down2_split) {
-        if ((rc = run_patchdown(h->down2, f2, B, S / 4, S / 4, 2 * C, 0, f3, s, "gemm_down2", next_dir(h)))) return rc;
+        if ((rc = run_patchdown(h->down2, f2, B, S / 4, S / 4, 2 * C, 0, f3, s, "gemm_down2", next_dir(h), prod_of(NUNIF_SWIN_PRODUCER_DOWN2)))) return rc;
     } else if ((rc = run_gemm(h->down2, f2, B, S / 2, S / 2, 2 * C, S / 4, S / 4, 2, 0, 0, 2, 0, 0, 0.f, nullptr, f3,
                               2 * C, 1, s, "gemm_down2", next_dir(h))))
         return rc;
-    if (h->down2_split && (rc = run_gemm(h->down2b, f2, B, S / 2, S / 2, 2 * C, S / 4, S / 4, 2, 1, 0, 2, 0, 0, 0.f, f3, f3,
-                                         2 * C, 1, s, "gemm_down2b", next_dir(h))))
+    if (h->down2_split && (rc = run_patchdown(h->down2b, f2, B, S / 4, S / 4, 2 * C, 1, f3, s, "gemm_down2b", next_dir(h),
+                                              prod_of(NUNIF_SWIN_PRODUCER_DOWN2), 1)))
         return rc;
     if ((rc = tap(h, "down2", f3, (size_t)B * (S / 4) * (S / 4) * 2 * C * 2, s))) return rc;
     if ((rc = run_stage(h, h->swin[2], f3, B, S / 4, 2 * C, s, "swin3", nullptr, skip_of(2)))) return rc;
-    if ((rc = run_patchup(h->up2, f3, B, S / 4, S / 4, 2 * C, f2, s, "gemm_up2", next_dir(h)))) return rc;
+    if ((rc = run_patchup(h->up2, f3, B, S / 4, S / 4, 2 * C, f2, s, "gemm_up2", next_dir(h), prod_of(NUNIF_SWIN_PRODUCER_UP2)))) return rc;
     if ((rc = tap(h, "up2", f2, (size_t)B * (S / 2) * (S / 2) * 2 * C * 2, s))) return rc;
     if ((rc = run_stage(h, h->swin[3], f2, B, S / 2, 2 * C, s, "swin4", nullptr, skip_of(3)))) return rc;
     f16 *top = f1;
@@ -635,7 +697,7 @@
         top = (f16 *)h->g1.p;
         if ((rc = run_linear(h->proj2, f1, B, S, S, 0, nullptr, top, s, "gemm_proj2", next_dir(h)))) return rc;
     }
-    if ((rc = run_patchup(h->up1, f2, B, S / 2, S / 2, h->top_dim, top, s, "gemm_up1", next_dir(h)))) return rc;
+    if ((rc = run_patchup(h->up1, f2, B, S / 2, S / 2, h->top_dim, top, s, "gemm_up1", next_dir(h), prod_of(NUNIF_SWIN_PRODUCER_UP1)))) return rc;
     if ((rc = tap(h, "up1", top, (size_t)B * S * S * h->top_dim * 2, s))) return rc;
     if (h->top_dim == 96 && h->swin[4].back().fast && h->to_image_chained && !h->taps_on) {
         TailToImage ti;
@@ -822,9 +884,23 @@
 
 static int skip_pad_level() {
     const char *v = getenv("NUNIF_SWIN_SKIP_PAD");
-    if (!v) return 2;
+    if (!v) return 3;
     const int l = atoi(v);
-    return l <= 0 ? 0 : (l == 1 ? 1 : 2);
+    return l <= 0 ? 0 : std::min(l, 3);
+}
+
+extern "C" int nunif_hip_swin_unet_down2_test(nunif_swin_unet *h, const void *a, void *out, int32_t B, int32_t Ho, int32_t Wo,
+                                              int32_t acc_form, void *stream) {
+    NUNIF_REQUIRE(h && a && out && B > 0 && Ho > 0 && Wo > 0 && h->down2_split, "down2_test: bad argument");
+    hipStream_t s = (hipStream_t)stream;
+    int rc;
+    if ((rc = run_patchdown(h->down2, (const f16 *)a, B, Ho, Wo, 2 * h->C, 0, (f16 *)out, s, "gemm_down2", 0))) return rc;
+    if (acc_form) {
+        NUNIF_REQUIRE(patchdown_acc_enabled(), "down2_test: the accumulating PatchDown form is switched off");
+        return run_patchdown(h->down2b, (const f16 *)a, B, Ho, Wo, 2 * h->C, 1, (f16 *)out, s, "gemm_down2b", 1, nullptr, 1);
+    }
+    return run_gemm(h->down2b, (const f16 *)a, B, 2 * Ho, 2 * Wo, 2 * h->C, Ho, Wo, 2, 1, 0, 2, 0, 0, 0.f, (const f16 *)out, out, 2 * h->C, 1, s,
+                    "gemm_down2b", 1);
 }
 
 extern "C" int nunif_hip_swin_unet_tail192_test(nunif_swin_unet *h, int32_t stage, int32_t block, const void *att, void *x,
```

Result: faster. 344.9 MPix/s, median of 6 (+1.3%).
